# Spijkervet/Context-Aware-Sequential-Recommendation

Measured on AMD Instinct MI355X. Metric: user-sequences/sec (fwd+bwd), higher is better.
Workload: dtype f32 (bf16x3 split MFMA in attention); 1 GPU; ml-1m-shaped synthetic (6040 users, 3416 items), cast_1 maxlen=200 hidden_units=50 num_blocks=2 num_heads=1 dropout=0.20, batch 128/GPU (global 128), fwd+bwd+dense TF-Adam per step; parallelism=dp1, hip_graph=True, steps_per_graph_launch=4, attn_precision=bf16x3

## Files before the change

### context-aware-sequential-recommendation_amd/build.py

```python
import glob
import hashlib
import json
import os
import re
import subprocess
import sys
from concurrent.futures import ThreadPoolExecutor

PKG = os.path.dirname(os.path.abspath(__file__))
ROOT = os.path.dirname(PKG)
CSRC = os.path.join(PKG, "csrc")
LIB = os.path.join(PKG, "libcastrec.so")
LIB_TL = os.path.join(PKG, "libcastrec_tl.so")
SOURCES = ["cr_base.hip", "cr_embed.hip", "cr_layernorm.hip", "cr_eltwise.hip", "cr_gemm.hip",
           "cr_attn_fwd.hip", "cr_attn_bwd.hip", "cr_attn_bwd1.hip", "cr_attn_wide.hip", "cr_attn_bf.hip", "cr_gemm_bf.hip", "cr_block.hip", "cr_stack.hip", "cr_stack_bwd.hip", "cr_stack_bwd1.hip", "cr_wide.hip", "cr_head.hip", "cr_adam.hip", "cr_tgrad.hip", "cr_topk.hip", "cr_ce.hip", "cr_dist.hip", "cr_sampler.cpp", "cr_index.cpp"]
FLAGS = ["--offload-arch=gfx950", "-O3", "-fPIC", "-std=c++17", "-I", os.path.join(ROOT, "include"), "-I", CSRC,
         "-Wall", "-Wno-unused-function",
         "-fno-slp-vectorize"]


ISA_CHECKED = ["cr_stack.hip", "cr_stack_bwd.hip", "cr_stack_bwd1.hip", "cr_wide.hip", "cr_attn_bf.hip",
               "cr_block.hip", "cr_attn_fwd.hip", "cr_attn_bwd.hip", "cr_attn_bwd1.hip", "cr_gemm.hip", "cr_gemm_bf.hip",
               "cr_topk.hip", "cr_ce.hip"]
SLP_PROTECTED = ("cr_stack", "cr_wide")
_PK_F32 = ("v_pk_fma_f32", "v_pk_mul_f32", "v_pk_add_f32")
_LABEL = re.compile(r"^([A-Za-z_$][\w$.]*):")
_MODIFIER = re.compile(r"\s(op_sel|op_sel_hi|neg_lo|neg_hi|clamp|mul:|div:|quad_perm|row_|bank_mask|bound_ctrl|dst_sel|dst_unused|src\d_sel)")


def _operands(rest):
    m = _MODIFIER.search(" " + rest)
    if m:
        rest = (" " + rest)[:m.start()]
    return [o.strip().lstrip("-").strip("|") for o in rest.split(",") if o.strip()]


_VREG = re.compile(r"^v(?:\[(\d+):(\d+)\]|(\d+))$")
_WRITES_VGPR = ("v_", "ds_read", "global_load", "buffer_load", "flat_load", "scratch_load")


def _vregs(op):
    m = _VREG.match(op)
    if not m:
        return frozenset()
    if m.group(3) is not None:
        return frozenset([int(m.group(3))])
    return frozenset(range(int(m.group(1)), int(m.group(2)) + 1))


def scan_isa(text):
    out = dict(kernels=0, pk_fma=0, pk_add=0, pk_mul=0, in_place_any=0, mfma={}, mixed_mfma_chains=0, violations=[])
    func, last = "?", []
    mfma_dst = {}
    for no, line in enumerate(text.splitlines(), 1):
        if line and not line[0].isspace():
            m = _LABEL.match(line)
            if m and not line.startswith("."):
                func, last, mfma_dst = m.group(1), [], {}
                out["kernels"] += 1
            continue
        t = line.strip()
        if not t.startswith(_WRITES_VGPR):
            continue
        mn, _, rest = t.partition(" ")
        ops = _operands(rest.split(";")[0])
        dst = ops[0] if ops else ""
        dregs = _vregs(dst)
        if mn.startswith("v_mfma"):
            out["mfma"][mn] = out["mfma"].get(mn, 0) + 1
            srcc = _vregs(ops[3]) if len(ops) >= 4 else frozenset()
            prev = mfma_dst.get(srcc)
            if prev and prev[0] != mn:
                out["mixed_mfma_chains"] += 1
                out["violations"].append((func, no, [prev[1], t]))
            for k in [k for k in mfma_dst if k & dregs]:
                del mfma_dst[k]
            if dregs:
                mfma_dst[dregs] = (mn, t)
        elif dregs and mfma_dst:
            for k in [k for k in mfma_dst if k & dregs]:
                del mfma_dst[k]
        if not t.startswith("v_"):
            continue
        if mn in _PK_F32:
            out[mn[2:-4]] += 1
            if dst in ops[1:]:
                out["in_place_any"] += 1
            if mn == "v_pk_fma_f32" and len(ops) >= 4 and ops[3] == dst:
                for pm, pd, pl in last:
                    if pm in _PK_F32 and pd == dst:
                        out["violations"].append((func, no, [pl, t]))
                        break
        last = (last + [(mn, dst, t)])[-2:]
    return out


def _source_digest(src, headers, flags):
    h = hashlib.sha256()
    for f in [src] + headers:
        with open(f, "rb") as fh:
            h.update(fh.read())
    h.update(" ".join(flags).encode())
    return h.hexdigest()


def isa_summary_path(source_name, timeline=False):
    return os.path.join(CSRC, "build_tl" if timeline else "build", source_name + ".isa.json")


def check_isa_file(source_name, flags, headers, hipcc=None, listing=None):
    src = os.path.join(CSRC, source_name)
    if listing is None:
        listing = os.path.join(CSRC, "build", source_name + ".s")
        cmd = [hipcc or _hipcc()] + flags + ["-x", "hip", "-S", "--cuda-device-only", src, "-o", listing]
        r = subprocess.run(cmd, capture_output=True, text=True)
        if r.returncode != 0:
            raise RuntimeError("compile failed: %s\n%s" % (" ".join(cmd), r.stderr))
    with open(listing) as fh:
        res = scan_isa(fh.read())
    res["source"], res["digest"], res["flags"] = source_name, _source_digest(src, headers, flags), flags
    with open(isa_summary_path(source_name), "w") as fh:
        json.dump(res, fh, indent=1)
    if res["violations"]:
        f, no, chain = res["violations"][0]
        raise RuntimeError("%s: %d forbidden instruction chains in the device code (in-place packed fp32, or MFMAs of two shapes on one accumulator; first: %s, line %d: %s) -- see build.py ISA_CHECKED"
                           % (source_name, len(res["violations"]), f, no, " ; ".join(chain)))
    return res


def isa_is_current(source_name, flags, headers):
    try:
        with open(isa_summary_path(source_name)) as fh:
            d = json.load(fh)
    except (OSError, ValueError):
        return False
    return d.get("digest") == _source_digest(os.path.join(CSRC, source_name), headers, flags) and not d.get("violations")


def file_flags(source_name, timeline=False):
    extra = os.environ.get("CASTREC_EXTRA_FLAGS", "").split()
    slp_ok = os.environ.get("CASTREC_SLP_FILES", "cr_attn_bf.hip").split()
    bad = [f for f in slp_ok if f.startswith(SLP_PROTECTED)]
    if bad:
        raise RuntimeError("CASTREC_SLP_FILES names %s: these sources are never compiled with SLP vectorisation "
                           "(profiles/r04_flake/README.md)" % bad)
    if any(f in ("-fslp-vectorize", "-fvectorize-slp") or f.startswith("-fslp-vectorize") for f in extra):
        raise RuntimeError("CASTREC_EXTRA_FLAGS may not re-enable SLP vectorisation (profiles/r04_flake/README.md)")
    flags = FLAGS + (["-DCR_TIMELINE=1"] if timeline else []) + extra
    return [f for f in flags if not (f == "-fno-slp-vectorize" and source_name in slp_ok)]


HEADERS = [os.path.join(CSRC, h) for h in ("cr_common.hpp", "cr_attn_common.hpp", "cr_bf16.hpp", "cr_rlayout.hpp", "cr_rbwd.hpp")] \
    + [os.path.join(ROOT, "include", "castrec.h")]
EXTRA_DEPS = {"cr_adam.hip": ["cr_tgrad.hpp"], "cr_tgrad.hip": ["cr_tgrad.hpp"]}


def _hipcc():
    for c in (os.environ.get("HIPCC"), "/opt/rocm/bin/hipcc", "hipcc"):
        if c and (os.path.isabs(c) and os.path.exists(c) or not os.path.isabs(c)):
            return c
    raise RuntimeError("hipcc not found")


def _stale(obj, srcs):
    if not os.path.exists(obj):
        return True
    t = os.path.getmtime(obj)
    return any(os.path.getmtime(s) > t for s in srcs)


def build(force=False, verbose=False, timeline=False):
    hipcc = _hipcc()
    bdir = "build_tl" if timeline else "build"
    lib = LIB_TL if timeline else LIB
    os.makedirs(os.path.join(CSRC, bdir), exist_ok=True)
    headers = HEADERS
    objs, jobs = [], []
    for s in SOURCES:
        src = os.path.join(CSRC, s)
        obj = os.path.join(CSRC, bdir, s + ".o")
        objs.append(obj)
        fl = file_flags(s, timeline)
        checked = s in ISA_CHECKED and not timeline
        deps = [src] + headers + [os.path.join(CSRC, h) for h in EXTRA_DEPS.get(s, [])]
        if checked and not force and not _stale(obj, deps) and not isa_is_current(s, fl, headers):
            force_this = True
        else:
            force_this = False
        if force or force_this or _stale(obj, deps):
            cmd = [hipcc] + fl + (["-save-temps=obj"] if checked else []) + (["-x", "hip"] if s.endswith(".hip") else []) + ["-c", src, "-o", obj]
            jobs.append((cmd, s if checked else None, fl))

    def run(job):
        cmd, checked_src, fl = job if isinstance(job, tuple) else (job, None, None)
        r = subprocess.run(cmd, capture_output=True, text=True)
        if r.returncode != 0:
            raise RuntimeError("compile failed: %s\n%s\n%s" % (" ".join(cmd), r.stdout, r.stderr))
        if verbose and r.stderr.strip():
            print(r.stderr, file=sys.stderr)
        if checked_src:
            stem = checked_src[:-4]
            bd = os.path.join(CSRC, bdir)
            try:
                check_isa_file(checked_src, fl, headers, listing=os.path.join(bd, stem + "-hip-amdgcn-amd-amdhsa-gfx950.s"))
            finally:
                for f in glob.glob(os.path.join(bd, stem + "-hip-amdgcn-*")) + glob.glob(os.path.join(bd, stem + "-host-*")) \
                        + glob.glob(os.path.join(bd, stem + ".hip-hip-*")):
                    os.remove(f)

    with ThreadPoolExecutor(max_workers=4) as ex:
        list(ex.map(run, jobs))
    if force or jobs or _stale(lib, objs):
        run(([hipcc, "--offload-arch=gfx950", "-shared", "-fPIC", "-o", lib] + objs + ["-lpthread"], None, None))
    return lib


if __name__ == "__main__":
    print(build(force="--force" in sys.argv, verbose=True, timeline="--timeline" in sys.argv))
```

### context-aware-sequential-recommendation_amd/csrc/cr_adam.hip

```cpp
#include <math.h>
#include <stdlib.h>
#include <string.h>

#include "cr_common.hpp"
#include "cr_tgrad.hpp"

int tg_unit_grid(const cr_tgrad_desc* d);

#define ADAM_COLS 256
#define ADAM_WAVES 16
typedef float f4a __attribute__((ext_vector_type(4), aligned(4)));
__device__ __forceinline__ float slab_sum256(const float* slabs, int n_slabs, int n_dense, int j0, float (*part)[ADAM_COLS]) {
    const int lane = threadIdx.x & 63, w = threadIdx.x >> 6;
    const int j = j0 + 4 * lane;
    f4a acc = (f4a){0.f, 0.f, 0.f, 0.f};
    if (j + 3 < n_dense) {
        for (int s0 = w; s0 < n_slabs; s0 += 16 * ADAM_WAVES) {
            f4a v[16];
            int cnt = 0;
#pragma unroll
            for (int u = 0; u < 16; ++u)
                if (s0 + ADAM_WAVES * u < n_slabs) { v[u] = *reinterpret_cast<const f4a*>(slabs + (size_t)(s0 + ADAM_WAVES * u) * n_dense + j); cnt = u + 1; }
#pragma unroll
            for (int u = 0; u < 16; ++u)
                if (u < cnt) acc += v[u];
        }
    } else {
        for (int s = w; s < n_slabs; s += ADAM_WAVES)
            for (int u = 0; u < 4; ++u)
                if (j + u < n_dense) acc[u] += slabs[(size_t)s * n_dense + j + u];
    }
    part[w][4 * lane + 0] = acc.x; part[w][4 * lane + 1] = acc.y; part[w][4 * lane + 2] = acc.z; part[w][4 * lane + 3] = acc.w;
    __syncthreads();
    float g = 0.0f;
    if (threadIdx.x < ADAM_COLS) {
#pragma unroll
        for (int k = 0; k < ADAM_WAVES; ++k) g += part[k][threadIdx.x];
    }
    return g;
}

template <bool STREAM, int LPR, int VEC>
__global__ __launch_bounds__(64 * ADAM_WAVES) void k_adam(cr_adam_desc d, cr_tgrad_desc g, int nb_dense, int nb_lazy, int nb_units, int nb_ring) {
    __shared__ float part_s[ADAM_WAVES * ADAM_COLS + 4];
    float (*part)[ADAM_COLS] = reinterpret_cast<float (*)[ADAM_COLS]>(part_s);
    constexpr bool TG = LPR > 0;
    cr_kernarg_touch<sizeof(cr_adam_desc) + (TG ? sizeof(cr_tgrad_desc) : 0)>();
    const uint32_t t = d.step_snapshot ? *d.step_snapshot : *reinterpret_cast<const uint32_t*>(d.state + 4);
    const int bid = (int)blockIdx.x;
    if (bid >= (int)gridDim.x - nb_ring) {
        constexpr int NT = 64 * ADAM_WAVES;
        const long long n_copy = d.ids_copy_elems ? d.ids_copy_elems : d.ids_slot_elems;
        const int32_t* src1 = d.ids_ring + (long long)((t + 1u) % (uint32_t)d.ids_ring_slots) * d.ids_slot_elems;
        const long long first = (long long)(bid - ((int)gridDim.x - nb_ring)) * NT + threadIdx.x, stride = (long long)nb_ring * NT;
        if ((d.ids_slot_elems & 3) == 0 && (n_copy & 3) == 0 && (((uintptr_t)d.ids_ring | (uintptr_t)d.ids_dst) & 15) == 0) {
            const int4* src = reinterpret_cast<const int4*>(src1);
            int4* dst = reinterpret_cast<int4*>(d.ids_dst);
            for (long long i = first; i < (n_copy >> 2); i += stride) dst[i] = src[i];
        } else {
            for (long long i = first; i < n_copy; i += stride) d.ids_dst[i] = src1[i];
        }
        return;
    }
    const float* st = d.stats ? d.stats : d.state;
    const float n = st[2];
    float inv_n = 0.0f, lr_t = 0.0f;
    auto scalars = [&]() {
        inv_n = n > 0.0f ? 1.0f / n : 0.0f;
        const float b1t = powf(d.beta1, (float)t), b2t = powf(d.beta2, (float)t);
        lr_t = d.lr * sqrtf(1.0f - b2t) / (1.0f - b1t);
    };
    auto update = [&](long long i, float g) {
        g *= inv_n;
        if (i < d.n_l2) g = fmaf(d.l2, d.p[i], g);
        const float m = d.beta1 * d.m[i] + (1.0f - d.beta1) * g;
        const float v = d.beta2 * d.v[i] + (1.0f - d.beta2) * g * g;
        d.m[i] = m;
        d.v[i] = v;
        d.p[i] -= lr_t * m / (sqrtf(v) + d.eps);
    };
    if (bid < nb_dense) {
        const int j0 = bid * ADAM_COLS;
        const int ns = d.slab_counts ? min(d.slab_counts[bid], d.n_slabs) : d.n_slabs;
        const bool mine = threadIdx.x < ADAM_COLS && j0 + (int)threadIdx.x < d.n_dense;
        const long long i = d.n_table + j0 + (mine ? (int)threadIdx.x : 0);
        const float p0 = mine ? d.p[i] : 0.0f, m0 = mine ? d.m[i] : 0.0f, v0 = mine ? d.v[i] : 0.0f;
        float g = slab_sum256(d.dense_slabs, ns, d.n_dense, j0, part);
        scalars();
        if (mine) {
            g *= inv_n;
            if (i < d.n_l2) g = fmaf(d.l2, p0, g);
            const float m = d.beta1 * m0 + (1.0f - d.beta1) * g;
            const float v = d.beta2 * v0 + (1.0f - d.beta2) * g * g;
            d.m[i] = m;
            d.v[i] = v;
            d.p[i] = p0 - lr_t * m / (sqrtf(v) + d.eps);
        }
    } else if (bid < nb_dense + nb_lazy) {
        const int lane = threadIdx.x & 63;
        const int W = nb_lazy * ADAM_WAVES;
        scalars();
        for (int k = (bid - nb_dense) * ADAM_WAVES + (threadIdx.x >> 6); k < d.n_lazy_ids; k += W) {
            const int id = d.lazy_ids[k];
            if (id <= 0 || id >= d.lazy_rows) continue;
            int mine = 0;
            if (lane == 0) mine = atomicExch(&d.lazy_flags[id], t) != t;
            mine = __shfl(mine, 0, 64);
            if (!mine) continue;
            for (int c = lane; c < d.lazy_D; c += 64) {
                const long long i = (long long)id * d.lazy_D + c;
                const float g = d.table_grad[i];
                d.table_grad[i] = 0.0f;
                update(i, g);
            }
        }
    } else if (TG && bid < nb_dense + nb_lazy + nb_units) {
        const int32_t* ix = tg_index(g, t);
        constexpr int W = TG ? VEC : 1;
        scalars();
        tg_unit_blocks<TG ? LPR : 16, W, (TG && VEC == 4) ? 8 : 16>(g, ix, bid - nb_dense - nb_lazy, nb_units, part_s,
            reinterpret_cast<int*>(part_s + ADAM_WAVES * ADAM_COLS),
            [&](int row, int col0, const float (&acc)[W]) {
                const long long i = (long long)row * g.D + col0;
                float p0[W], m0[W], v0[W];
                tg_load<W>(p0, d.p + i); tg_load<W>(m0, d.m + i); tg_load<W>(v0, d.v + i);
#pragma unroll
                for (int u = 0; u < W; ++u) {
                    float gu = acc[u] * inv_n;
                    if (i + u < d.n_l2) gu = fmaf(d.l2, p0[u], gu);
                    m0[u] = d.beta1 * m0[u] + (1.0f - d.beta1) * gu;
                    v0[u] = d.beta2 * v0[u] + (1.0f - d.beta2) * gu * gu;
                    p0[u] -= lr_t * m0[u] / (sqrtf(v0[u]) + d.eps);
                }
                tg_store<W>(d.m + i, m0); tg_store<W>(d.v + i, v0); tg_store<W>(d.p + i, p0);
            });
    } else if (TG) {
        const int32_t* ix = tg_index(g, t);
        const uint32_t* bits = reinterpret_cast<const uint32_t*>(ix + ix[6]);
        const int nb_table = gridDim.x - nb_dense - nb_lazy - nb_units - nb_ring;
        const int tb = bid - nb_dense - nb_lazy - nb_units;
        constexpr int NT = 64 * ADAM_WAVES;
        const long long stride = (long long)nb_table * NT;
        auto touched = [&](uint32_t row) { return ((bits[row >> 5] >> (row & 31)) & 1u) != 0u; };
        scalars();
        if ((g.D & 3) == 0) {
            const float b1 = d.beta1, b2 = d.beta2, c1 = 1.0f - d.beta1, c2 = 1.0f - d.beta2;
            auto ld4 = [](const float* q) { return STREAM ? __builtin_nontemporal_load(reinterpret_cast<const f4a*>(q)) : *reinterpret_cast<const f4a*>(q); };
            auto st4 = [](float* q, const f4a x) {
                if (STREAM) __builtin_nontemporal_store(x, reinterpret_cast<f4a*>(q));
                else *reinterpret_cast<f4a*>(q) = x;
            };
            const long long n4 = d.n_table >> 2;
            const unsigned D4 = (unsigned)g.D >> 2;
            const int sh = (D4 & (D4 - 1u)) == 0u ? __builtin_ctz(D4) : -1;
            constexpr int U = 4;
            for (long long q = (long long)tb * NT + threadIdx.x; q < n4; q += U * stride) {
                bool in[U];
                uint32_t bw[U];
                uint32_t row[U];
                f4a p[U], m[U], v[U];
#pragma unroll
                for (int u = 0; u < U; ++u) {
                    const long long qq = q + u * stride;
                    in[u] = qq < n4;
                    const long long qc = in[u] ? qq : q;
                    row[u] = sh >= 0 ? (uint32_t)(qc >> sh) : (uint32_t)((unsigned long long)qc / D4);
                    bw[u] = bits[row[u] >> 5];
                    p[u] = ld4(d.p + 4 * qc); m[u] = ld4(d.m + 4 * qc); v[u] = ld4(d.v + 4 * qc);
                }
#pragma unroll
                for (int u = 0; u < U; ++u) {
                    if (!in[u] || ((bw[u] >> (row[u] & 31)) & 1u)) continue;
                    const long long i = 4 * (q + u * stride);
                    f4a po;
#pragma unroll
                    for (int e = 0; e < 4; ++e) {
                        float gu = 0.0f;
                        if (i + e < d.n_l2) gu = fmaf(d.l2, p[u][e], gu);
                        m[u][e] = b1 * m[u][e] + c1 * gu;
                        v[u][e] = b2 * v[u][e] + c2 * gu * gu;
                        po[e] = p[u][e] - lr_t * m[u][e] / (sqrtf(v[u][e]) + d.eps);
                    }
                    st4(d.m + i, m[u]); st4(d.v + i, v[u]); st4(d.p + i, po);
                }
            }
        } else {
            for (long long i = (long long)tb * NT + threadIdx.x; i < d.n_table; i += stride)
                if (!touched((uint32_t)((unsigned long long)i / (unsigned)g.D))) update(i, 0.0f);
        }
    } else {
        const int nb_table = gridDim.x - nb_dense - nb_lazy - nb_ring;
        const int tb = bid - nb_dense - nb_lazy;
        const long long first = nb_lazy > 0 ? (long long)d.lazy_rows * d.lazy_D : 0;
// ... 189 lines not shown
```

### context-aware-sequential-recommendation_amd/csrc/cr_stack_bwd1.hip

```cpp
#include <math.h>
#include <stdlib.h>
#include <string.h>
#include <type_traits>
#include <mutex>

#include "cr_rbwd.hpp"

#define B1_DRAIN() asm volatile("s_waitcnt vmcnt(0)" ::: "memory")
#define B1_NT_WS true
#define B1_ROWS 224
#define B1_FSTR (B1_ROWS * 64)

#define DS_EXACT(DS) ((DS) > 0 ? ((DS) & 255) : (DS))
#define DS_D(DS, run) ((DS) > 0 ? ((DS) & 255) : (run))
#define B1_NKT(DS, a) ((DS) > 255 ? (((DS) >> 8) & 255) : (a).nkt)
#define B1_T(DS, a) ((DS) > 65535 ? ((DS) >> 16) : (a).T)
#undef D_NF
#define D_NF(DS) ((DS) > 0 ? ((DS) & 255) / 16 : ((DS) < 0 ? -(DS) - 1 : -1))

struct B1Args {
    cr_block_bwd_desc bd;
    cr_attn_desc ad;
    cr_embed_bwd_desc sc;
    cr_ln_bwd_desc ln;
    const float* dy2;
    float* dx2;
    const float* ln_dy2;
    float* d_addend2;
    float* sbuf; float* sbuf2;
    int B, T, nkt, scatter, has_ln;
    int small;
    int n0, add;
    float isd, isd_log2e, invT;
    unsigned qpk[8], kpk[8];
    unsigned long long* ts;
};

__device__ __forceinline__ const B1Args& b1_args_again() {
    auto p = __builtin_amdgcn_kernarg_segment_ptr();
    asm volatile("" : "+s"(p));
    return *reinterpret_cast<const B1Args*>((const void*)p);
}

#ifdef CR_TIMELINE
#define B1_TS(slot)                                                                                          \
    do {                                                                                                     \
        if (a.ts && (threadIdx.x & 63) == 0) {                                                               \
            unsigned long long* ts_ = a.ts + (((size_t)blockIdx.y * gridDim.x + blockIdx.x) * SB_WAVES + (threadIdx.x >> 6)) * 32; \
            ts_[(slot)] = ((slot) == 0 || (slot) == 31) ? wall_clock64() : clock64();                        \
            if ((slot) == 0) ts_[30] = clock64();          \
            if ((slot) == 31) ts_[29] = clock64();                                                           \
        }                                                                                                    \
    } while (0)
#else
#define B1_TS(slot) do { } while (0)
#endif

template <bool SPLIT>
struct B1Lds {
    static constexpr int NIMG = SPLIT ? 4 : 2;
    static constexpr int WST = SPLIT ? 2 * ST_WIMG : ST_WIMG;
    static constexpr int IST = SPLIT ? 2 * SB_IMG : SB_IMG;
    static constexpr int MATB = (SPLIT ? 2 : 1) * B1_FSTR * 2;
    static constexpr int LOB = B1_FSTR * 2;
    static constexpr int W_OFF = NIMG * B1_FSTR;
    static constexpr int F_OFF_BYTES = (W_OFF + 2 * WST) * 2;
    static constexpr int GAM = 0, GAMF = 64, PART = 128, PARTF = PART + 2 * SB_WAVES * 64, SDEL = PARTF + 2 * SB_WAVES * 64,
                         KB = SDEL + 2 * B1_ROWS, SMX = KB, SUNI = SMX + 2 * B1_ROWS, SQV = SUNI + B1_ROWS,
                         TFLAG = SQV + B1_ROWS, NFLOAT = TFLAG + 16;
    static_assert(SUNI >= KB + B1_ROWS + 16, "the key bias (one extra tile) inside the shared floats");
    static constexpr int BYTES = F_OFF_BYTES + NFLOAT * 4;
};

template <bool BIAS = false>
__device__ __forceinline__ void b1_wstore(float* dst, int ldw, float* bias_dst, const f32x4 (&acc)[2], const f32x4 (&accb)[2], int D, int it, int jt0, bool add) {
    const int lane = threadIdx.x & 63, li = lane & 15, lg = lane >> 4;
#pragma unroll
    for (int j = 0; j < 2; ++j) {
        const int col = 16 * (jt0 + j) + li;
#pragma unroll
        for (int r = 0; r < 4; ++r) {
            const int k = 16 * it + 4 * lg + r;
            if (col < D && (BIAS ? k < D : k <= D)) {
                float* p = (k < D) ? dst + (size_t)k * ldw + col : bias_dst + col;
                __builtin_nontemporal_store(add ? *p + acc[j][r] : acc[j][r], p);
            }
        }
        if (BIAS && it == 0 && lg == 0 && col < D) bias_dst[col] = add ? bias_dst[col] + accb[j][0] : accb[j][0];
    }
}
__device__ __forceinline__ void b1_ln_fold(float* part, const f32x4 (&ag)[4], const f32x4 (&ab)[4]) {
    const int lane = lane_now(), wave = __builtin_amdgcn_readfirstlane(threadIdx.x >> 6), lg = lane >> 4;
    float u[16];
#pragma unroll
    for (int ct = 0; ct < 4; ++ct)
#pragma unroll
        for (int r = 0; r < 4; ++r) {
            float x = ag[ct][r];
            asm volatile("s_nop 1\n\t"
                         "v_add_f32_dpp %0, %0, %0 row_mirror row_mask:0xf bank_mask:0x3\n\t"
                         "v_add_f32_dpp %0, %1, %1 row_mirror row_mask:0xf bank_mask:0xc"
                         : "+v"(x) : "v"(ab[ct][r]));
            u[4 * ct + r] = x;
        }
#pragma unroll
    for (int j = 0; j < 8; ++j)
        asm volatile("s_nop 1\n\t"
                     "v_add_f32_dpp %0, %0, %0 row_half_mirror row_mask:0xf bank_mask:0x5\n\t"
                     "v_add_f32_dpp %0, %1, %1 row_half_mirror row_mask:0xf bank_mask:0xa"
                     : "+v"(u[j]) : "v"(u[8 + j]));
    const bool b1 = (lane & 2) != 0, b0 = (lane & 1) != 0;
    float w[4], z[2];
#pragma unroll
    for (int j = 0; j < 4; ++j) {
        const float keep = b1 ? u[4 + j] : u[j], send = b1 ? u[j] : u[4 + j];
        w[j] = keep + __int_as_float(__builtin_amdgcn_update_dpp(0, __float_as_int(send), 0x1B, 0xF, 0xF, false));
    }
#pragma unroll
    for (int j = 0; j < 2; ++j) {
        const float keep = b0 ? w[2 + j] : w[j], send = b0 ? w[j] : w[2 + j];
        z[j] = keep + __int_as_float(__builtin_amdgcn_update_dpp(0, __float_as_int(send), 0xB1, 0xF, 0xF, false));
    }
    const int col = 16 * (((lane >> 2) & 1) * 2 + ((lane >> 1) & 1)) + 4 * lg + 2 * (lane & 1);
    float* dst = part + ((lane & 8) ? SB_WAVES * 64 : 0) + wave * 64 + col;
    *reinterpret_cast<float2*>(dst) = make_float2(z[0], z[1]);
}
template <int NSET = 1>
__device__ __forceinline__ void b1_ln_flush(const float* part, float* dg, float* db, int D, bool add) {
    for (int c = threadIdx.x; c < D; c += SB_NT) {
        float g = 0.0f, b = 0.0f;
#pragma unroll
        for (int s = 0; s < NSET; ++s)
#pragma unroll
            for (int w = 0; w < SB_WAVES; ++w) { g += part[(2 * s * SB_WAVES + w) * 64 + c]; b += part[((2 * s + 1) * SB_WAVES + w) * 64 + c]; }
        dg[c] = add ? dg[c] + g : g;
        db[c] = add ? db[c] + b : b;
    }
}

struct B1Steps { uint32_t ffn2, attn, emb; };
struct B1Acc { f32x4 aw1[2], aw2[2], aw1b[2], aw2b[2], ag[4], ab[4], agF[4], abF[4]; };

template <bool SPLIT, int DS, bool QSIDE, int HD, class F>
__device__ __forceinline__ void b1_phase1(const B1Args& a, unsigned char* smem, int n, B1Acc& A, B1Steps& steps, F&& before_last_products) {
    constexpr bool BIAS = DS_EXACT(DS) == 64;
    constexpr bool LATE_Q = !QSIDE && (HD == 2 || DS_EXACT(DS) > 50 || DS <= 0);
    typedef B1Lds<SPLIT> L;
    const cr_block_bwd_desc& bd = a.bd;
    const cr_block_desc& d = bd.f;
    __bf16* Im = reinterpret_cast<__bf16*>(smem);
    __bf16* Wi = Im + L::W_OFF;
    float* fl = reinterpret_cast<float*>(smem + L::F_OFF_BYTES);
    float* gam = fl + L::GAM; float* gamF = fl + L::GAMF; float* part = fl + L::PART; float* partF = fl + L::PARTF; float* sdel = fl + L::SDEL;
    constexpr int WST = L::WST, IST = L::IST;
    const int D = DS_D(DS, d.D), T = B1_T(DS, a);
    const DCtx dcx = d_ctx<D_NF(DS)>(D);
    const int wave = __builtin_amdgcn_readfirstlane(threadIdx.x >> 6);
    uint32_t sv_ffn2 = cr_step_request(d.drop_ffn2), sv_attn = cr_step_request(a.ad.drop), sv_emb = a.scatter ? cr_step_request(a.sc.f.drop) : 0u;
    const float scale1 = (d.drop_ffn1.rate > 0.0f) ? 1.0f / (1.0f - d.drop_ffn1.rate) : 1.0f;
    B1_TS(13);
    f32x4 (&aw1)[2] = A.aw1; f32x4 (&aw2)[2] = A.aw2; f32x4 (&ag)[4] = A.ag; f32x4 (&ab)[4] = A.ab; f32x4 (&agF)[4] = A.agF; f32x4 (&abF)[4] = A.abF;
    f32x4 (&aw1b)[2] = A.aw1b; f32x4 (&aw2b)[2] = A.aw2b;
#pragma unroll
    for (int j = 0; j < 2; ++j) { aw1[j] = (f32x4){0.f, 0.f, 0.f, 0.f}; aw2[j] = aw1[j]; aw1b[j] = aw1[j]; aw2b[j] = aw1[j]; }
#pragma unroll
    for (int ct = 0; ct < 4; ++ct) { ag[ct] = (f32x4){0.f, 0.f, 0.f, 0.f}; ab[ct] = ag[ct]; agF[ct] = ag[ct]; abF[ct] = ag[ct]; }
    const int it = wave >> 1, jt0 = 2 * (wave & 1);
    RRaw rdy, rdy2, rhid, rfin, ro, rq, ry;
    const size_t MD = (size_t)d.M * D;
    auto tile_rows = [&](int rd, int& m, bool& rok) {
        const int q = 16 * (rd * SB_TPR + wave) + (lane_now() & 15);
        rok = q < T;
        m = n * T + min(q, T - 1);
    };
    auto issue_a = [&](int rd) {
        if (rd * SB_TPR < B1_NKT(DS, a) && wave < min(SB_TPR, B1_NKT(DS, a) - rd * SB_TPR)) {
            int m; bool rok;
            tile_rows(rd, m, rok);
            const u32 mo = (u32)m * (u32)(4 * D);
            if (a.has_ln) {
                r_issue(rdy, a.ln.dy, (u32)m * (u32)(4 * a.ln.lddy), dcx, rok);
                if (a.ln_dy2) r_issue(rdy2, a.ln_dy2, (u32)m * (u32)(4 * a.ln.lddy), dcx, rok);
                r_issue(ry, d.y, mo, dcx);
            } else {
                r_issue(rdy, bd.dy, mo, dcx);
                if (a.dy2) r_issue(rdy2, a.dy2, mo, dcx);
            }
            r_issue(rhid, d.hid, mo, dcx);
// ... 849 lines not shown
                    d4[t2] = *reinterpret_cast<const float4*>(vq + 64 * t2 + 4 * B1_ROWS * h);
                    w4[t2] = *reinterpret_cast<const float4*>(vq + 64 * t2 + 4 * (L::SQV - L::SDEL));
                }
                constexpr int JB = (SPLIT || HD == 2) ? 2 : 4;
                const int jbase = HD == 2 ? 2 * h : 0;
                bf8 oth[JB], otl[JB];
#pragma unroll
                for (int jt = 0; jt < JB; ++jt) {
                    oth[jt] = trF(L::MATB, jbase + jt, 0);
                    otl[jt] = SPLIT ? trF(L::MATB, jbase + jt, 1) : oth[jt];
                }
                float xa[8], xd[8];
                const uint32_t xb_h = xbase + (uint32_t)h * xhead;
                auto finish = [&](auto diag_c, int t2, int xo, const f32x4& s, const f32x4& p) {
                    constexpr bool DIAG = decltype(diag_c)::value;
                    const int lt = 2 * qp + t2;
                    const float mm[4] = {m4[t2].x, m4[t2].y, m4[t2].z, m4[t2].w}, dd[4] = {d4[t2].x, d4[t2].y, d4[t2].z, d4[t2].w}, ww[4] = {w4[t2].x, w4[t2].y, w4[t2].z, w4[t2].w};
                    const uint32_t x0 = xb_h + (uint32_t)lt * (16u * xT);
                    const float bias = (lt < kt) ? -INFINITY : kbias;
                    float pn[4], w[4];
#pragma unroll
                    for (int r = 0; r < 4; ++r) {
                        pn[r] = __builtin_amdgcn_exp2f(fmaf(s[r], a.isd_log2e, -mm[r]) + bias);
                        if (DIAG) pn[r] = (lt != kt || key <= 16 * lt + 4 * lg + r) ? pn[r] : 0.0f;
                        w[r] = (cr_mix(x0 + (uint32_t)r * xT) >= dc.thresh) ? ww[r] : 0.0f;
                        xd[xo + r] = pn[r] * (p[r] * w[r] - dd[r]);
                    }
                    if ((uni_m >> lt) & 1u) {
                        const float4 u4 = *reinterpret_cast<const float4*>(vq + 64 * t2 + 4 * (L::SUNI - L::SDEL));
                        const float uu[4] = {u4.x, u4.y, u4.z, u4.w};
#pragma unroll
                        for (int r = 0; r < 4; ++r) xa[xo + r] = (pn[r] + key_in_T * uu[r]) * w[r];
                    } else {
#pragma unroll
                        for (int r = 0; r < 4; ++r) xa[xo + r] = pn[r] * w[r];
                    }
                };
                if (qp == (kt >> 1)) {
                    finish(std::true_type{}, 0, 0, s0, p0);
                    finish(std::true_type{}, 1, 4, s1, p1);
                } else {
                    finish(std::false_type{}, 0, 0, s0, p0);
                    finish(std::false_type{}, 1, 4, s1, p1);
                }
                bf8 ah, al, dh, dl;
                split8<SPLIT>(xa, ah, al);
                split8<SPLIT>(xd, dh, dl);
#pragma unroll
                for (int jt = 0; jt < JB; ++jt) dv[jbase + jt] = mma<SPLIT>(oth[jt], otl[jt], ah, al, dv[jbase + jt]);
                if (HD == 1) {
#pragma unroll
                    for (int j0 = JB; j0 < 4; j0 += JB) {
#pragma unroll
                        for (int jt = 0; jt < JB; ++jt) {
                            oth[jt] = trF(L::MATB, j0 + jt, 0);
                            otl[jt] = SPLIT ? trF(L::MATB, j0 + jt, 1) : oth[jt];
                        }
#pragma unroll
                        for (int jt = 0; jt < JB; ++jt) dv[j0 + jt] = mma<SPLIT>(oth[jt], otl[jt], ah, al, dv[j0 + jt]);
                        BF_SGB(0x100, (SPLIT ? 4 : 2) * JB, 0);
                        BF_SGB(0x008, (SPLIT ? 3 : 1) * JB, 0);
                    }
                }
#pragma unroll
                for (int j0 = jbase; j0 < (HD == 2 ? jbase + 2 : 4); j0 += JB) {
#pragma unroll
                    for (int jt = 0; jt < JB; ++jt) {
                        oth[jt] = trF(0, j0 + jt, 0);
                        otl[jt] = SPLIT ? trF(0, j0 + jt, 1) : oth[jt];
                    }
#pragma unroll
                    for (int jt = 0; jt < JB; ++jt) dk[j0 + jt] = mma<SPLIT>(oth[jt], otl[jt], dh, dl, dk[j0 + jt]);
                    BF_SGB(0x100, (SPLIT ? 4 : 2) * JB, 0);
                    BF_SGB(0x008, (SPLIT ? 3 : 1) * JB, 0);
                }
            }
        }
#pragma unroll
        for (int jt = 0; jt < 4; ++jt) dk[jt] *= a.isd;
        if (ti == 0) B1_TS(6);
        if (ti == 0 && (int)((tpk >> 5) & 31u) < B1_NKT(DS, a)) issue_tile((int)((tpk >> 5) & 31u));
        const B1Args& ar = b1_args_again();
        r_store<B1_NT_WS>(const_cast<float*>(ar.bd.dqkv) + MD, mo, dk, rok, dcx);
        r_store<B1_NT_WS>(const_cast<float*>(ar.bd.dqkv) + 2 * MD, mo, dv, rok, dcx);
        f32x4 dxp[4];
        {
            bf8 gh[2], gl[2];
            r_split<SPLIT>(dk, gh, gl);
            r_gemm_t<SPLIT, false>(dxp, Wi, Wi + ST_WIMG, gh, gl);
            r_split<SPLIT>(dv, gh, gl);
            r_gemm_t<SPLIT, true>(dxp, Wi + WST, Wi + WST + ST_WIMG, gh, gl);
        }
        if (ar.scatter) {
            b1_scatter_prep(ar, dxp, m, rok, D, steps.emb);
            r_store(ar.sbuf2, mo, dxp, rok, dcx);
        } else {
            r_store(ar.dx2, mo, dxp, rok, dcx);
        }
    }
    B1_TS(4);
    __builtin_amdgcn_s_setprio(0);
    B1_DRAIN();
    __syncthreads();
    B1_TS(7);
    f32x4 awk[2], awv[2], awkb[2], awvb[2];
#pragma unroll
    for (int j = 0; j < 2; ++j) { awk[j] = (f32x4){0.f, 0.f, 0.f, 0.f}; awv[j] = awk[j]; awkb[j] = awk[j]; awvb[j] = awk[j]; }
    const int it = wave >> 1, jt0 = 2 * (wave & 1);
    const int R = B1_NKT(DS, a) > SB_TPR ? 2 : 1;
    RRaw r1, r2, r3;
    auto issue3 = [&](int rd) {
        if (rd < R && wave < min(SB_TPR, B1_NKT(DS, a) - rd * SB_TPR)) {
            const int qq = 16 * (rd * SB_TPR + wave) + (lane_now() & 15);
            const u32 mo = (u32)(base_row + min(qq, T - 1)) * (u32)(4 * D);
            r_issue(r1, bk.x, mo, dcx);
            r_issue(r2, dKg, mo, dcx, qq < T);
            r_issue(r3, dVg, mo, dcx, qq < T);
        }
    };
    issue3(0);
    B1Small small;
#pragma unroll 1
    for (int rd = 0; rd < R; ++rd) {
        const int ntr = min(SB_TPR, B1_NKT(DS, a) - rd * SB_TPR);
        if (wave < ntr) {
            f32x4 x[4], g[4];
            r_finish(x, r1, dcx);
            plant_one(x, D);
            img_put<SPLIT>(Im, Im + SB_IMG, 16 * wave, x);
            r_finish(g, r2, dcx);
            img_put<SPLIT>(Im + IST, Im + IST + SB_IMG, 16 * wave, g);
            r_finish(g, r3, dcx);
            img_put<SPLIT>(Im + 2 * IST, Im + 2 * IST + SB_IMG, 16 * wave, g);
        }
        issue3(rd + 1);
        if (rd == R - 1 && a.scatter && a.small) b1_small_issue<D_NF(DS)>(small, a, a.sbuf2, n, D);
        __syncthreads();
        if (rd == 0) B1_TS(16);
        wgrad_accum<SPLIT, BIAS>(awk, awkb, Im, Im + SB_IMG, Im + IST, Im + IST + SB_IMG, ntr, it, jt0);
        wgrad_accum<SPLIT, BIAS>(awv, awvb, Im, Im + SB_IMG, Im + 2 * IST, Im + 2 * IST + SB_IMG, ntr, it, jt0);
        __syncthreads();
        if (rd == 0) B1_TS(19);
    }
    B1_TS(17);
    const size_t so = (size_t)blockIdx.x * bd.slab_stride;
    b1_wstore<BIAS>(bd.g_wqkv + so + D, 3 * D, bd.g_bqkv + so + D, awk, awkb, D, it, jt0, add);
    b1_wstore<BIAS>(bd.g_wqkv + so + 2 * D, 3 * D, bd.g_bqkv + so + 2 * D, awv, awvb, D, it, jt0, add);
    B1_TS(18);
    if (a.scatter && a.small) b1_small_table<SPLIT, D_NF(DS)>(a, smem, reinterpret_cast<int*>(fl + L::PART), small, n, D, add);
    else if (a.scatter) b1_scatter_rows(a, a.sbuf2, n, D);
    B1_TS(5);
}

template <bool SPLIT, int DS, int HD>
__global__ __launch_bounds__(SB_NT) void k_stack_block_bwd(B1Args a) {
    extern __shared__ __attribute__((aligned(16))) unsigned char smem_raw[];
    B1_TS(0);
    cr_kernarg_touch<sizeof(B1Args)>();
    B1_TS(15);
    const int n = a.n0 + (int)blockIdx.x;
    if (blockIdx.y == 0) {
        B1Acc acc;
        B1Steps steps;
        b1_phase1<SPLIT, DS, false, HD>(a, smem_raw, n, acc, steps, [] {});
        b1_k_side<SPLIT, DS, HD>(a, smem_raw, n, a.add != 0, acc, steps);
    } else {
        B1Acc acc;
        B1Stage st;
        WRegs<1, SB_NT> w;
        B1Steps steps;
        b1_phase1<SPLIT, DS, true, HD>(a, smem_raw, n, acc, steps, [&] { b1_q_stage_issue<DS>(a, n, st, w); });
        b1_q_side<SPLIT, DS, HD>(a, smem_raw, n, a.add != 0, acc, steps, st, w);
    }
    B1_TS(31);
}

struct B1Deal { unsigned pk[8]; bool done; };
static void b1_deal_search(int nkt, bool query_pass, unsigned (&pk)[8]) {
    int wave_of[16], order[16];
    cr_deal_search(nkt, query_pass, wave_of, order);
    for (int w = 0; w < 8; ++w) pk[w] = 0x3FFu;
    int wc[8] = {0, 0, 0, 0, 0, 0, 0, 0};
    for (int k = 0; k < nkt; ++k) {
        const int t = order[k], w = wave_of[t];
        pk[w] = (pk[w] & ~(31u << (5 * wc[w]))) | ((unsigned)t << (5 * wc[w]));
        ++wc[w];
    }
}
static void b1_deal_tiles(int nkt, bool query_pass, unsigned (&pk)[8]) {
    static B1Deal cache[2][16];
    static std::mutex mu;
    {
        std::lock_guard<std::mutex> lock(mu);
        B1Deal& c = cache[query_pass ? 1 : 0][nkt & 15];
        if (!c.done) { b1_deal_search(nkt, query_pass, c.pk); c.done = true; }
        for (int w = 0; w < 8; ++w) pk[w] = c.pk[w];
    }
    if (const char* ov = getenv(query_pass ? "CASTREC_B1_QPK" : "CASTREC_B1_KPK")) {
        unsigned t[8];
        int w = 0;
        const char* c = ov;
        while (w < 8 && *c) {
            unsigned a0 = 31, a1 = 31;
            if (*c != '-') { a0 = (unsigned)strtol(c, const_cast<char**>(&c), 10); if (*c == ':') { ++c; a1 = (unsigned)strtol(c, const_cast<char**>(&c), 10); } }
            else ++c;
            t[w++] = (a0 & 31u) | ((a1 & 31u) << 5);
            if (*c == ',') ++c;
        }
        if (w == 8) for (int i = 0; i < 8; ++i) pk[i] = t[i];
    }
}

extern "C" int cr_stack_block_bwd_deal(int nkt, int query_pass, uint32_t* pk) {
    CR_REQUIRE(pk && nkt >= 1 && nkt <= 2 * SB_TPR, "cr_stack_block_bwd_deal: 1 <= tiles <= 14");
    unsigned t[8];
    b1_deal_tiles(nkt, query_pass != 0, t);
    for (int w = 0; w < 8; ++w) pk[w] = t[w];
    return CR_OK;
}

static const char* b1_unsupported(const cr_block_bwd_desc* bd, const cr_attn_desc* ad, int B, int T, int precision) {
    if (!bd || !ad) return "NULL description";
    const cr_block_desc& d = bd->f;
    const bool two_heads = d.D == 64 && ad->H == 2 && ad->d == 32;
    if (!two_heads && (d.D < 8 || d.D >= 64)) return "hidden size 8..63 (one head), or 64 with two heads of 32";
    if (precision != CR_PREC_BF16X3 && precision != CR_PREC_BF16) return "bf16 arithmetic (precision) only";
    if (B < 1 || T < 1 || d.M != B * T) return "M = B T";
    if ((T + 15) / 16 > 2 * SB_TPR) return "T <= 224 (two rounds of 7 row tiles)";
    if ((size_t)d.M * d.D * 4 >= ((size_t)1 << 32)) return "activations of 4 GiB or more (32-bit row offsets)";
    if (bd->n_slabs < 1) return "n_slabs";
    if (!two_heads && (ad->H != 1 || ad->d != d.D)) return "one head of d = D (or two heads of 32 at D = 64)";
    if (ad->B != B || ad->T != T) return "the block's B and T";
    if (ad->ld != d.D || ad->Q != d.qkv || ad->K != d.qkv + (size_t)d.M * d.D || ad->V != d.qkv + 2 * (size_t)d.M * d.D) return "Q / K / V = the parts of the block's qkv";
    if (ad->residual != d.q_in || ad->out != d.o || ad->k_valid != d.k_valid || ad->q_valid != d.q_valid) return "the attention call of this block (residual = q_in, out = o, masks)";
    if (!ad->row_stats) return "row_stats (saved by the forward)";
    if (ad->attn_weights) return "attention weights are not taken";
    return nullptr;
}
extern "C" int cr_stack_block_bwd_supported(const cr_block_bwd_desc* bd, const cr_attn_desc* ad, int B, int T, int precision) {
    return b1_unsupported(bd, ad, B, T, precision) == nullptr;
}

template <bool SPLIT, int DS, int HD = 1>
static int launch_b1(B1Args& a, int nwg, hipStream_t s) {
    static cr_devmask attr = 0;
    int rc = cr_raise_lds_limit(reinterpret_cast<const void*>(&k_stack_block_bwd<SPLIT, DS, HD>), &attr);
    if (rc) return rc;
    for (int n0 = 0; n0 < a.B; n0 += nwg) {
        a.n0 = n0;
        a.add = n0 > 0;
        hipLaunchKernelGGL((k_stack_block_bwd<SPLIT, DS, HD>), dim3(a.B - n0 < nwg ? a.B - n0 : nwg, 2), dim3(SB_NT), B1Lds<SPLIT>::BYTES, s, a);
    }
    return cr_check_launch("cr_stack_block_bwd");
}

extern "C" int cr_stack_block_bwd(const cr_block_bwd_desc* bd, const cr_attn_desc* ad, const cr_block_bwd1_ext* x, const cr_ln_bwd_desc* lnf,
                                  const cr_embed_bwd_desc* sc, int B, int T, int precision, void* stream) {
    const char* why = b1_unsupported(bd, ad, B, T, precision);
    CR_REQUIRE(why == nullptr, "cr_stack_block_bwd: unsupported (%s)", why ? why : "");
    CR_REQUIRE(x != nullptr, "cr_stack_block_bwd: NULL extension");
    B1Args a;
    memset(static_cast<void*>(&a), 0, sizeof(a));
    a.bd = *bd; a.ad = *ad;
    a.B = B; a.T = T; a.nkt = (T + 15) / 16;
    const cr_block_desc* d = &bd->f;
    CR_REQUIRE(bd->d_o && bd->dqkv && d->hid && d->f_in && d->o && d->q_in && d->x && d->mask_ids && d->w1 && d->w2 && d->wqkv && d->ln1_g && d->ln2_g,
               "cr_stack_block_bwd: NULL pointer");
    CR_REQUIRE(bd->g_w1 && bd->g_b1 && bd->g_w2 && bd->g_b2 && bd->g_ln2_g && bd->g_ln2_b && bd->g_wqkv && bd->g_bqkv && bd->g_ln1_g && bd->g_ln1_b,
               "cr_stack_block_bwd: NULL gradient pointer");
    CR_REQUIRE(bd->dq_part == nullptr, "cr_stack_block_bwd: dq_part is not taken");
    a.dy2 = x->dy2; a.dx2 = x->dx2; a.ln_dy2 = x->lnf_dy2; a.d_addend2 = x->d_addend2;
    if (lnf) {
        CR_REQUIRE(lnf->x == d->y && lnf->ldx == d->D && lnf->M == d->M && lnf->D == d->D, "cr_stack_block_bwd: the LayerNorm's input must be this block's y");
        CR_REQUIRE(lnf->gamma && lnf->dy && lnf->dgamma && lnf->dbeta && lnf->accumulate == 0, "cr_stack_block_bwd: LayerNorm backward arguments");
        CR_REQUIRE(lnf->slab_stride == bd->slab_stride && lnf->n_slabs == bd->n_slabs, "cr_stack_block_bwd: the LayerNorm's slabs must be the block's");
        CR_REQUIRE((size_t)lnf->M * lnf->lddy * 4 < ((size_t)1 << 32), "cr_stack_block_bwd: dy of 4 GiB or more");
        a.ln = *lnf;
        a.has_ln = 1;
    } else {
        CR_REQUIRE(bd->dy, "cr_stack_block_bwd: dy is NULL");
        CR_REQUIRE(x->lnf_dy2 == nullptr, "cr_stack_block_bwd: lnf_dy2 without a LayerNorm");
    }
    if (sc) {
        const cr_embed_desc* e = &sc->f;
        CR_REQUIRE(e->ids && e->M == d->M && e->D == d->D && e->ld_out == d->D && e->col_off == 0 && e->T > 0 && e->V > 0,
                   "cr_stack_block_bwd: the embedding recipe must describe the block's dense input x");
        CR_REQUIRE(!bd->dx_accumulate, "cr_stack_block_bwd: dx_accumulate with a scatter (this kernel must be the only producer of dx)");
        if (sc->n_slabs > 0) {
            const int nw = B < bd->n_slabs ? B : bd->n_slabs;
            CR_REQUIRE(sc->table_grad && !sc->pos_grad && e->V <= 256 && sc->n_slabs >= 2 * nw,
                       "cr_stack_block_bwd: small-table scatter needs table_grad, no pos_grad, V <= 256 and n_slabs >= 2 * min(B, n_slabs of the block)");
            a.small = 1;
        }
        CR_REQUIRE(sc->d_addend == nullptr || (e->ld_add == d->D && x->d_addend2 != nullptr), "cr_stack_block_bwd: d_addend must be dense [M, D] and come with d_addend2");
        a.sc = *sc;
        a.scatter = 1;
        a.sbuf = sc->d_addend ? sc->d_addend : bd->dx;
        a.sbuf2 = sc->d_addend ? x->d_addend2 : x->dx2;
        CR_REQUIRE(a.sbuf && a.sbuf2 && a.sbuf != a.sbuf2, "cr_stack_block_bwd: the scatter needs two [M, D] row buffers (d_addend + d_addend2, or dx + dx2)");
    } else {
        CR_REQUIRE(bd->dx && x->dx2 && bd->dx != x->dx2, "cr_stack_block_bwd: dx / dx2");
    }
    a.isd = 1.0f / sqrtf((float)ad->d);
    a.isd_log2e = a.isd * 1.4426950408889634f;
    a.invT = 1.0f / (float)T;
    b1_deal_tiles(a.nkt, true, a.qpk);
    b1_deal_tiles(a.nkt, false, a.kpk);
    a.ts = g_attn_ts_which == 9 ? g_attn_ts : nullptr;
    if (a.ts) {
        static const char* only = getenv("CASTREC_TS_LAUNCH");
        static unsigned long long* seen_for = nullptr;
        static int count = 0;
        if (seen_for != a.ts) { seen_for = a.ts; count = 0; }
        if (only && atoi(only) != count) a.ts = nullptr;
        ++count;
    }
    const int nwg = B < bd->n_slabs ? B : bd->n_slabs;
    const bool split = precision == CR_PREC_BF16X3;
    hipStream_t s = cr_stream(stream);
    switch (d->D) {
    case 64: return split ? launch_b1<true, 64, 2>(a, nwg, s) : launch_b1<false, 64, 2>(a, nwg, s);
    case 50:
        static const bool no_nk = getenv("CASTREC_B1_NO_NKT") != nullptr;
        if (a.T == 200 && !no_nk) return split ? launch_b1<true, 50 | (13 << 8) | (200 << 16)>(a, nwg, s) : launch_b1<false, 50 | (13 << 8) | (200 << 16)>(a, nwg, s);
        return split ? launch_b1<true, 50>(a, nwg, s) : launch_b1<false, 50>(a, nwg, s);
    case 32: return split ? launch_b1<true, 32>(a, nwg, s) : launch_b1<false, 32>(a, nwg, s);
    case 40: return split ? launch_b1<true, 40>(a, nwg, s) : launch_b1<false, 40>(a, nwg, s);
    case 48: return split ? launch_b1<true, 48>(a, nwg, s) : launch_b1<false, 48>(a, nwg, s);
    case 56: return split ? launch_b1<true, 56>(a, nwg, s) : launch_b1<false, 56>(a, nwg, s);
    default: break;
    }
    switch (d->D / 16) {
    case 0: return split ? launch_b1<true, -1>(a, nwg, s) : launch_b1<false, -1>(a, nwg, s);
    case 1: return split ? launch_b1<true, -2>(a, nwg, s) : launch_b1<false, -2>(a, nwg, s);
    case 2: return split ? launch_b1<true, -3>(a, nwg, s) : launch_b1<false, -3>(a, nwg, s);
    default: return split ? launch_b1<true, -4>(a, nwg, s) : launch_b1<false, -4>(a, nwg, s);
    }
}
```

### context-aware-sequential-recommendation_amd/engine.py

```python
import ctypes as C
import math
import os
import zlib

import numpy as np
import torch

from . import lib as L
from . import ops as O

ATTN_PRECISIONS = {"f32": L.PREC_F32, "bf16x3": L.PREC_BF16X3, "bf16": L.PREC_BF16}
DEFAULT_ATTN_PRECISION = "bf16x3"
LOSSES = ("bce", "ce")
ALL_LOSSES = LOSSES + ("sampled_ce", "gbce")
SOFTMAX_LOSSES = ("ce", "sampled_ce", "gbce")
SAMPLED_LOSSES = ("sampled_ce", "gbce")
CE_PROPOSALS = ("uniform", "popularity")

MODELS = ["cast_1", "cast_2", "cast_3", "cast_4", "cast_5", "cast_6", "cast_7", "cast_8", "cast_9",
          "sasrec", "sasrec_static"]


def site_id(name):
    return zlib.crc32(name.encode()) & 0xFFFFFF


def positional_encoding(dim, length):
    v = np.array([pos / np.power(10000, 2 * i / dim) for pos in range(length) for i in range(dim)])
    v[::2] = np.sin(v[::2])
    v[1::2] = np.cos(v[1::2])
    return v.reshape(length, dim).astype(np.float32)


class Hyper:

    def __init__(self, args=None, **kw):
        d = dict(maxlen=50, hidden_units=50, num_blocks=2, num_heads=1, dropout_rate=0.5, l2_emb=0.0, lr=1e-3,
                 max_bins=200, num_context_blocks=2, seed=42, loss="bce", ce_negatives=256, gbce_t=0.75, ce_proposal="uniform",
                 ce_pop_power=1.0)
        for k in d:
            if args is not None and hasattr(args, k):
                d[k] = getattr(args, k)
        d.update(kw)
        self.__dict__.update(d)
        if self.hidden_units % self.num_heads != 0:
            raise ValueError("hidden_units must be divisible by num_heads (tf.split, modules.py:208)")


def auto_slabs(M):
    n = -(-M // 128)
    if n < 128:
        n = -(-M // 64)
    return max(1, min(256, n))


def _stack_entries(prefix, L_, D):
    out = []
    for i in range(L_):
        p = "%s.%d." % (prefix, i)
        out += [(p + "ln1.gamma", (D,), "ones"), (p + "ln1.beta", (D,), "zeros"),
                (p + "wqkv", (D, 3 * D), "glorot3"), (p + "bqkv", (3 * D,), "zeros"),
                (p + "ln2.gamma", (D,), "ones"), (p + "ln2.beta", (D,), "zeros"),
                (p + "w1", (D, D), "glorot"), (p + "b1", (D,), "zeros"),
                (p + "w2", (D, D), "glorot"), (p + "b2", (D,), "zeros")]
    out += [(prefix + ".lnf.gamma", (D,), "ones"), (prefix + ".lnf.beta", (D,), "zeros")]
    return out


def model_structure(model, hp):
    L_, Lc = hp.num_blocks, hp.num_context_blocks
    s = dict(ctx={}, small=[], mlp=0, learned_pos=model in ("sasrec", "cast_9"))
    if model in ("cast_1", "cast_2", "cast_3", "cast_4", "cast_5", "cast_6"):
        s["ctx"]["ctx_time"] = L_
    if model == "cast_8":
        s["ctx"].update(ctx_hours=L_, ctx_days=L_)
    if model == "cast_9":
        s["ctx"].update(ctx_hours=Lc, ctx_days=Lc, ctx_time=Lc)
    if "ctx_time" in s["ctx"]:
        s["small"].append(("time_emb", hp.max_bins + 1))
    if model in ("cast_3", "cast_4", "cast_5", "cast_6", "cast_7", "cast_8", "cast_9"):
        s["small"] += [("hours_emb", 25), ("days_emb", 8)]
    s["mlp"] = {"cast_2": 2, "cast_3": 3, "cast_4": 4, "cast_5": 3, "cast_6": 4, "cast_7": 3, "cast_8": 3, "cast_9": 4}.get(model, 0)
    return s


class ParamLayout:
    def __init__(self, model, usernum, itemnum, hp):
        D, T = hp.hidden_units, hp.maxlen
        st = model_structure(model, hp)
        table = [("item_emb", (itemnum + 1, D), "glorot")]
        if st["learned_pos"]:
            table.append(("pos_emb", (T, D), "glorot"))
        dense = [(n, (v, D), "glorot") for n, v in st["small"]]
        for pfx, Lc in st["ctx"].items():
            dense += _stack_entries(pfx, Lc, D)
        if st["mlp"]:
            k = st["mlp"]
            dense += [("mlp.w1", (k * D, k * D), "glorot"), ("mlp.b1", (k * D,), "zeros"),
                      ("mlp.w2", (k * D, D), "glorot"), ("mlp.b2", (D,), "zeros")]
        dense += _stack_entries("trunk", hp.num_blocks, D)
        self.entries, off = {}, 0
        for (n, shape, init) in table:
            self.entries[n] = (off, shape, init, "table"); off += int(np.prod(shape))
        self.n_table = off
        for (n, shape, init) in dense:
            self.entries[n] = (off, shape, init, "dense"); off += int(np.prod(shape))
        self.n_total, self.n_dense, self.D = off, off - self.n_table, D
        self.n_l2 = self.n_table + sum(int(np.prod(self.entries[n][1])) for n, _ in st["small"])

    def logical_names(self):
        out = []
        for n in self.entries:
            if n.endswith("wqkv"):
                out += [n[:-4] + x for x in ("wq", "wk", "wv")]
            elif n.endswith("bqkv"):
                out += [n[:-4] + x for x in ("bq", "bk", "bv")]
            else:
                out.append(n)
        return out

    def view(self, flat, name):
        D = self.D
        for j, x in enumerate(("q", "k", "v")):
            if name.endswith(".w" + x):
                off, shape, _, _ = self.entries[name[:-2] + "wqkv"]
                return flat[off:off + D * 3 * D].view(D, 3 * D)[:, j * D:(j + 1) * D]
            if name.endswith(".b" + x):
                off, shape, _, _ = self.entries[name[:-2] + "bqkv"]
                return flat[off + j * D:off + (j + 1) * D]
        off, shape, _, _ = self.entries[name]
        return flat[off:off + int(np.prod(shape))].view(*shape)

    def init_host(self, seed):
        rs = np.random.RandomState(seed)
        flat = np.zeros(self.n_total, np.float32)
        for n, (off, shape, init, _) in self.entries.items():
            size = int(np.prod(shape))
            if init == "glorot":
                lim = math.sqrt(6.0 / (shape[0] + shape[1]))
                flat[off:off + size] = rs.uniform(-lim, lim, size)
            elif init == "glorot3":
                D = shape[0]
                lim = math.sqrt(6.0 / (D + D))
                flat[off:off + size] = rs.uniform(-lim, lim, size)
            elif init == "ones":
                flat[off:off + size] = 1.0
        return flat


class Engine:
    def __init__(self, model, usernum, itemnum, hp, batch_size, training=True, seed=None, n_slabs=None,
                 share=None, batch_global=None, row_offset=0, want_attn=False, device="cuda", fused=None,
                 attn_precision=None, lazy_adam=None, loss=None, ce_negatives=None, gbce_t=None, ce_proposal=None):
        if model not in MODELS:
            raise ValueError("model must be one of %s" % MODELS)
        if not torch.cuda.is_available():
            raise RuntimeError("castrec_amd needs a ROCm GPU (gfx950); there is no CPU fallback")
        self.model, self.hp, self.B, self.T, self.D = model, hp, batch_size, hp.maxlen, hp.hidden_units
        self.H = hp.num_heads
        if attn_precision is None:
            attn_precision = os.environ.get("CASTREC_ATTN_PRECISION") or getattr(hp, "attn_precision", None) or DEFAULT_ATTN_PRECISION
        if attn_precision not in ATTN_PRECISIONS:
            raise ValueError("attn_precision must be one of %s" % sorted(ATTN_PRECISIONS))
        self.attn_precision = attn_precision
        if attn_precision == "f32" and hp.hidden_units > 64:
            import warnings
            warnings.warn("attn_precision='f32' at hidden_units %d leaves the tuned path: the exact-fp32 row phases above 64 columns are "
                          "the unfused kernels (2.6x slower at the C4 shape, 11x at C5; profiles/r02d_other_shapes.log); the "
                          "fp32-grade default is 'bf16x3'" % hp.hidden_units, RuntimeWarning, stacklevel=2)
        self.lazy_adam = bool(int(os.environ.get("CASTREC_LAZY_ADAM", "0"))) if lazy_adam is None else bool(lazy_adam)
        if loss is None:
            loss = getattr(hp, "loss", None) or "bce"
        if loss not in ALL_LOSSES:
            raise ValueError("loss must be one of %s, got %r" % (ALL_LOSSES, loss))
        self.loss = loss if training else "bce"
        if ce_negatives is None:
            ce_negatives = getattr(hp, "ce_negatives", None) or 256
        self.ce_negatives = int(ce_negatives)
        if gbce_t is None:
            gbce_t = getattr(hp, "gbce_t", None)
            gbce_t = 0.75 if gbce_t is None else gbce_t
        self.gbce_t = float(gbce_t)
        if ce_proposal is None:
            ce_proposal = getattr(hp, "ce_proposal", None) or "uniform"
        if ce_proposal not in CE_PROPOSALS:
            raise ValueError("ce_proposal must be one of %s, got %r" % (CE_PROPOSALS, ce_proposal))
        self.ce_proposal = ce_proposal if training else "uniform"
        if self.ce_proposal == "popularity" and self.loss != "sampled_ce":
            raise ValueError("ce_proposal='popularity' needs loss='sampled_ce', got loss=%r (gbce's beta is derived for uniform "
                             "sampling; bce and ce draw no shared negatives)" % self.loss)
        if self.loss in SOFTMAX_LOSSES:
            op = {"ce": "cr_softmax_ce", "sampled_ce": "cr_sampled_ce", "gbce": "cr_gbce"}[self.loss]
            if self.lazy_adam:
                raise ValueError("loss='%s' does not take row-sparse Adam (lazy_adam): every item row has a gradient" % self.loss)
            if (batch_global is not None and batch_global != batch_size) or row_offset:
                raise ValueError("loss='%s' does not take data parallelism (the item table's gradient is not in the exchanged bucket)"
                                 % self.loss)
            if not 8 <= hp.hidden_units <= 256:
                raise ValueError("loss='%s' needs 8 <= hidden_units <= 256 (%s), got %d" % (self.loss, op, hp.hidden_units))
        if self.loss in SAMPLED_LOSSES and not 1 <= self.ce_negatives <= L.CR_SCE_MAX_SAMPLES:
            raise ValueError("loss='%s' needs 1 <= ce_negatives <= %d (%s), got %d"
                             % (self.loss, L.CR_SCE_MAX_SAMPLES, op, self.ce_negatives))
        if self.loss == "gbce":
            if not 0.0 <= self.gbce_t <= 1.0:
                raise ValueError("loss='gbce' needs 0 <= gbce_t <= 1, got %r" % (gbce_t,))
            alpha = min(1.0, self.ce_negatives / max(1, itemnum - 1))
            self.gbce_beta = 1.0 - self.gbce_t * (1.0 - alpha)
        self.M = self.B * self.T
        self.usernum, self.itemnum = usernum, itemnum
        self.training = training
        self.single_pass_bwd = os.environ.get("CASTREC_TWO_PASS_ATTN_BWD") != "1"
        self.fuse_tails = os.environ.get("CASTREC_NO_TAILS") != "1"
        self.fuse_embed = os.environ.get("CASTREC_NO_EMBED_FUSION") != "1"
        self.fuse_stack = os.environ.get("CASTREC_NO_STACK_KERNEL") != "1"
        self.fuse_stack_bwd = os.environ.get("CASTREC_NO_STACK_BWD") != "1"
        self.fuse_wide = os.environ.get("CASTREC_NO_WIDE") != "1"
        self._pending_embed = {}
        self._scatter_recipe, self._scatter_claimed = {}, set()
        self._ln_recipe, self._ln_claimed = {}, set()
        self._lnf_intent = {}
        self.fuse_block_bwd = os.environ.get("CASTREC_NO_BLOCK_BWD") != "1"
        self._grad2 = {}
        self._grad2_bufs = {}
        self._block_bwd_ranges = []
        self.fuse_head_ln = os.environ.get("CASTREC_NO_HEAD_LN") != "1" and self.loss == "bce"
        self._check_ids = os.environ.get("CASTREC_NO_ID_CHECK") != "1"
        self.fused = (4 <= hp.hidden_units <= 64) if fused is None else bool(fused)
        if self.fused and not 4 <= hp.hidden_units <= 64:
            raise ValueError("fused block kernels need 4 <= hidden_units <= 64")
        self.dev = torch.device(device)
        self.seed = hp.seed if seed is None else seed
        self.layout = share.layout if share is not None else ParamLayout(model, usernum, itemnum, hp)
        lay = self.layout
        if not n_slabs:
            n_slabs = auto_slabs(batch_size * hp.maxlen)
            if (self.fused and self.attn_precision != "f32" and 8 <= self.D <= 64 and self.T <= 224
                    and os.environ.get("CASTREC_NO_STACK_BWD") != "1"):
                items = batch_size * (2 if self.T > 112 else 1)
                if n_slabs < items <= 512:
                    n_slabs = items
                if (training and self.T > 16 and batch_size <= 160 and n_slabs < 2 * batch_size <= 512
                        and os.environ.get("CASTREC_NO_HEAD_FUSION") != "1"):
                    n_slabs = 2 * batch_size
        self.n_slabs = n_slabs
        self.n_wslabs = n_slabs if (self.fused or self.D <= 128) else min(n_slabs, int(os.environ.get("CASTREC_WSLABS", "32")))
        self._wgrad_ranges = []
        self.slab_counts = None
        f32 = dict(dtype=torch.float32, device=self.dev)
        if share is not None:
            self.P = share.P
        else:
            self.P = torch.from_numpy(lay.init_host(self.seed)).to(self.dev)
        self.state = torch.zeros(L.CR_STATE_FLOATS, **f32)
        self.state[4:5].view(torch.int32)[0] = 1
        if training:
            self.Mom = torch.zeros(lay.n_total, **f32)
            self.Vel = torch.zeros(lay.n_total, **f32)
            self.Gflat = torch.zeros(lay.n_total + 4, **f32)
            self.Gt = self.Gflat[:lay.n_table]
            self.Gs = torch.zeros(n_slabs, max(lay.n_dense, 1), **f32)
            if self.loss in SOFTMAX_LOSSES:
                nb = (O.softmax_ce_workspace_bytes(self.M, itemnum + 1, self.D) if self.loss == "ce"
                      else O.sampled_ce_workspace_bytes(self.M, self.ce_negatives, self.D) if self.loss == "sampled_ce"
                      else O.gbce_workspace_bytes(self.M, self.ce_negatives, self.D))
                self._ce_ws = torch.empty(nb, dtype=torch.uint8, device=self.dev)
            if self.loss in SAMPLED_LOSSES:
                self.samples = torch.zeros(self.ce_negatives, dtype=torch.int32, device=self.dev)
            if self.ce_proposal == "popularity":
                self.item_cdf = torch.zeros(itemnum + 1, dtype=torch.int32, device=self.dev)
                self.item_logq = torch.zeros(itemnum + 1, **f32)
                self._have_item_weights = False
        self.drop = O.Drop(hp.dropout_rate if training else 0.0, self.seed, self.state, row_offset)
        self.batch_global = self.B if batch_global is None else batch_global
        self.want_attn = want_attn
        self.attn_weights = None
        self._bufs, self._keep = {}, []
        self.fwd, self.bwd = [], []
        self._bwd_factories = []
        self._grad_written = set()
        i32 = dict(dtype=torch.int32, device=self.dev)
        self.ID_KEYS = ("seq", "pos", "neg", "time", "hours", "days")
        ng, ent = C.c_int(0), C.c_int(0)
        self.use_index = bool(training and not self.lazy_adam and self.loss == "bce" and os.environ.get("CASTREC_NO_INDEX") != "1"
                              and L.lib.cr_tgrad_geometry(self.D, C.byref(ng), C.byref(ent)))
        self.ids_words = 6 * self.M
        self.index_off = (self.ids_words + 3) // 4 * 4
        self.index_lay, self._ixb = None, None
        if self.use_index:
            self.index_lay = L.IndexLayout()
            t_pos = self.T if "pos_emb" in self.layout.entries else 0
            L.check(L.lib.cr_batch_index_layout(self.M, itemnum + 1, t_pos, ng.value, ent.value, C.byref(self.index_lay)), "cr_batch_index_layout")
            self._ixb = L.lib.cr_index_builder_create(self.M, itemnum + 1, t_pos, ng.value, ent.value)
            if not self._ixb:
                raise MemoryError("cr_index_builder_create(%d, %d, %d)" % (self.M, itemnum + 1, t_pos))
            self._tg_part = torch.zeros(self.index_lay.cap_blocks, (self.D + 3) // 4 * 4, dtype=torch.float32, device=self.dev)
            self._tg_tickets = torch.zeros(self.index_lay.cap_blocks, dtype=torch.int32, device=self.dev)
        self.slot_words = self.index_off + (int(self.index_lay.total_words) if self.use_index else 0) if self.use_index else self.ids_words
        self.batch_buf = torch.zeros(self.slot_words, **i32)
        self.ids_all = self.batch_buf[:self.ids_words].view(6, self.M)
        self.ids = {k: self.ids_all[i] for i, k in enumerate(self.ID_KEYS)}
        self._host_slot = np.zeros(self.slot_words, np.int32)
        self._tg_rows = None
        self.bitwise_reproducible = self.use_index
        self.static_pe = torch.from_numpy(positional_encoding(self.D, self.T)).to(self.dev)
        self._build()
        self._finalize()
        self.graph = None
        self._id_ring, self._ring_next = None, None

    def buf(self, name, cols, rows=None):
        if name not in self._bufs:
            self._bufs[name] = torch.zeros(self.M if rows is None else rows, cols, dtype=torch.float32, device=self.dev)
        return self._bufs[name]

    def vec(self, name, n=None):
        if name not in self._bufs:
            self._bufs[name] = torch.zeros(self.M if n is None else n, dtype=torch.float32, device=self.dev)
        return self._bufs[name]

    def p(self, name):
        return self.layout.view(self.P, name)

    def _pptr(self, name):
        off = self.layout.entries[name][0]
        return self.P.data_ptr() + 4 * off

    def _gptr(self, name):
        off, _, _, kind = self.layout.entries[name]
        if kind == "table":
            return self.Gt.data_ptr() + 4 * off
        return self.Gs.data_ptr() + 4 * (off - self.layout.n_table)

    def _acc(self, key):
        first = key not in self._grad_written
        self._grad_written.add(key)
        return 0 if first else 1

    def _call(self, lst, name, *args):
        if name in ("cr_gemm_rows", "cr_gemm_wgrad"):
            for i in range(args[1]):
                args[0][i].precision = ATTN_PRECISIONS[self.attn_precision]
        if name == "cr_gemm_wgrad":
            args = args[:3] + (self.n_wslabs,)
            base = self.Gs.data_ptr()
            for i in range(args[1]):
                w = args[0][i]
                o = (w.dW - base) // 4
                self._wgrad_ranges += [(o + k * w.ldw, o + k * w.ldw + w.N) for k in range(w.K)]
                if w.db:
                    self._wgrad_ranges.append(((w.db - base) // 4, (w.db - base) // 4 + w.N))
        fn = getattr(L.lib, name)
        self._keep.append(args)
        lst.append((name, fn, args))

    def rng(self, site_name, enabled=True):
        return self.drop.rng(site_id(site_name), enabled and self.training)

    def op_embed(self, ids_key, table, out, ld_out, col_off, scale, pos=None, addend=None, drop_site=None,
                 mask=False, small=False, into_stack=False):
        V, D = self.layout.entries[table][1]
        pos_ptr = None
        if pos == "static":
            pos_ptr = self.static_pe.data_ptr()
        elif pos == "learned":
            pos_ptr = self._pptr("pos_emb")
        add_buf = addend[0] if addend else None
        d = L.EmbedDesc(self.ids[ids_key].data_ptr(), self._pptr(table), self.M, self.T, D, V, 1, float(scale), pos_ptr,
                        add_buf.data_ptr() if addend else None, add_buf.shape[1] if addend else 0,
                        self.rng(drop_site) if drop_site else O.NO_DROP,
                        self.ids["seq"].data_ptr() if mask else None, out.data_ptr(), ld_out, col_off)
        if into_stack and self.fused and self.fuse_embed and ld_out == D and col_off == 0:
            self._pending_embed[out.data_ptr()] = d
        else:
            self._call(self.fwd, "cr_embed_fwd", C.byref(d))
        if not self.training:
            return

# ... 209 lines not shown
                G = self._gptr
                bbd = L.BlockBwdDesc(L.BlockDesc.from_buffer_copy(wbd), dy.data_ptr(), do.data_ptr(), dqkv.data_ptr(), dx.data_ptr(),
                                     self._acc(id(dx)), G(pfx + "ln1.gamma"), G(pfx + "ln1.beta"), G(pfx + "wqkv"), G(pfx + "bqkv"),
                                     G(pfx + "ln2.gamma"), G(pfx + "ln2.beta"), G(pfx + "w1"), G(pfx + "b1"), G(pfx + "w2"), G(pfx + "b2"),
                                     S, self.n_slabs)
                own_w = D == 128 and os.environ.get("CASTREC_WIDE_NO_WGRAD") != "1"
                if not own_w:
                    bbd.g_w1 = bbd.g_b1 = bbd.g_w2 = bbd.g_b2 = bbd.g_wqkv = bbd.g_bqkv = None
                dh = D // H
                fuse_attn = (T <= 256 and 8 <= dh <= 64 and dh % 16 == 0 and os.environ.get("CASTREC_WIDE_NO_DELTA") != "1"
                             and os.environ.get("CASTREC_BF_TWO_KERNELS") is None)
                if fuse_attn:
                    delta = self.vec("attn_delta_heads", H * M)
                    bbd.attn_delta = delta.data_ptr()
                self._call(lst, "cr_wide_ln_ffn_bwd", C.byref(bbd), g2.data_ptr(), g1.data_ptr(), H if fuse_attn else 0, prec)
                if not own_w:
                    w = (L.WgradDesc * 2)(L.WgradDesc(hid.data_ptr(), D, g2.data_ptr(), D, G(pfx + "w2"), D, G(pfx + "b2"), M, D, D),
                                          L.WgradDesc(f_in.data_ptr(), D, g1.data_ptr(), D, G(pfx + "w1"), D, G(pfx + "b1"), M, D, D))
                    self._call(lst, "cr_gemm_wgrad", w, 2, S, self.n_slabs)
                dq, dk, dv = dqkv.data_ptr(), dqkv.data_ptr() + MD4, dqkv.data_ptr() + 2 * MD4
                abd = L.AttnBwdDesc(L.AttnDesc.from_buffer_copy(ad), do.data_ptr(), D, dq, dk, dv, D, stats.data_ptr())
                if fuse_attn:
                    abd.delta = delta.data_ptr()
                self._call(lst, "cr_attn_bwd", C.byref(abd))
                if not own_w:
                    gw, gb = G(pfx + "wqkv"), G(pfx + "bqkv")
                    w2 = (L.WgradDesc * 3)(L.WgradDesc(q_in.data_ptr(), D, dq, D, gw, 3 * D, gb, M, D, D),
                                           L.WgradDesc(x.data_ptr(), D, dk, D, gw + 4 * D, 3 * D, gb + 4 * D, M, D, D),
                                           L.WgradDesc(x.data_ptr(), D, dv, D, gw + 8 * D, 3 * D, gb + 8 * D, M, D, D))
                    self._call(lst, "cr_gemm_wgrad", w2, 3, S, self.n_slabs)
                self._call(lst, "cr_wide_ln_qkv_bwd", C.byref(bbd), prec)
                return lst
            e = L.EltDesc(L.ELT_GRADPREP, dy.data_ptr(), D, None, 0, g2.data_ptr(), D, M, D, self.rng(pfx[:-1] + ".ffn2"), ids.data_ptr(), 0)
            self._call(lst, "cr_eltwise", C.byref(e))
            b = O.gemm_desc(g2, D, None, D, g1, D, M, D, D, trans_b=True)
            b.B = self._pptr(pfx + "w2")
            self._call(lst, "cr_gemm_rows", (L.GemmDesc * 1)(b), 1)
            e1 = L.EltDesc(L.ELT_GRADPREP, g1.data_ptr(), D, hid.data_ptr(), D, g1.data_ptr(), D, M, D, self.rng(pfx[:-1] + ".ffn1"), None, 0)
            self._call(lst, "cr_eltwise", C.byref(e1))
            w = (L.WgradDesc * 2)(L.WgradDesc(hid.data_ptr(), D, g2.data_ptr(), D, self._gptr(pfx + "w2"), D, self._gptr(pfx + "b2"), M, D, D),
                                  L.WgradDesc(f_in.data_ptr(), D, g1.data_ptr(), D, self._gptr(pfx + "w1"), D, self._gptr(pfx + "b1"), M, D, D))
            self._call(lst, "cr_gemm_wgrad", w, 2, S, self.n_slabs)
            b1 = O.gemm_desc(g1, D, None, D, df, D, M, D, D, trans_b=True, residual=dy, ldr=D, mask_ids=ids)
            b1.B = self._pptr(pfx + "w1")
            self._call(lst, "cr_gemm_rows", (L.GemmDesc * 1)(b1), 1)
            l2 = L.LnBwdDesc(o.data_ptr(), D, self._pptr(pfx + "ln2.gamma"), df.data_ptr(), D, do.data_ptr(), D, 0,
                             self._gptr(pfx + "ln2.gamma"), self._gptr(pfx + "ln2.beta"), S, self.n_slabs, M, D, 1e-8)
            self._call(lst, "cr_layernorm_bwd", C.byref(l2))
            dq, dk, dv = dqkv.data_ptr(), dqkv.data_ptr() + MD4, dqkv.data_ptr() + 2 * MD4
            abd = L.AttnBwdDesc(L.AttnDesc.from_buffer_copy(ad), do.data_ptr(), D, dq, dk, dv, D, stats.data_ptr())
            self._call(lst, "cr_attn_bwd", C.byref(abd))
            gw = self._gptr(pfx + "wqkv"); gb = self._gptr(pfx + "bqkv")
            w2 = (L.WgradDesc * 3)(L.WgradDesc(q_in.data_ptr(), D, dq, D, gw, 3 * D, gb, M, D, D),
                                   L.WgradDesc(x.data_ptr(), D, dk, D, gw + 4 * D, 3 * D, gb + 4 * D, M, D, D),
                                   L.WgradDesc(x.data_ptr(), D, dv, D, gw + 8 * D, 3 * D, gb + 8 * D, M, D, D))
            self._call(lst, "cr_gemm_wgrad", w2, 3, S, self.n_slabs)
            bq = O.gemm_desc(None, D, None, 3 * D, dq_in, D, M, D, D, trans_b=True, residual=do, ldr=D)
            bq.A, bq.B = dq, wqkv
            bk = O.gemm_desc(None, D, None, 3 * D, dx, D, M, D, D, trans_b=True, accumulate=bool(self._acc(id(dx))))
            bk.A, bk.B = dk, wqkv + 4 * D
            self._call(lst, "cr_gemm_rows", (L.GemmDesc * 2)(bq, bk), 2)
            bv = O.gemm_desc(None, D, None, 3 * D, dx, D, M, D, D, trans_b=True, accumulate=True)
            bv.A, bv.B = dv, wqkv + 8 * D
            self._call(lst, "cr_gemm_rows", (L.GemmDesc * 1)(bv), 1)
            l1 = L.LnBwdDesc(x.data_ptr(), D, self._pptr(pfx + "ln1.gamma"), dq_in.data_ptr(), D, dx.data_ptr(), D, 1,
                             self._gptr(pfx + "ln1.gamma"), self._gptr(pfx + "ln1.beta"), S, self.n_slabs, M, D, 1e-8)
            self._call(lst, "cr_layernorm_bwd", C.byref(l1))
            return lst
        self._bwd_factories.append(factory)

    def _block_desc(self, x, y, pfx):
        M, D = self.M, self.D
        q_in, o, f_in, hid = (self.buf(pfx + n, D) for n in ("q_in", "o", "f_in", "hid"))
        qkv = self.buf(pfx + "qkv", D, rows=3 * M)
        kvalid, qvalid = self.vec(pfx + "kvalid"), self.vec(pfx + "qvalid")
        P = self._pptr
        return L.BlockDesc(M, D, P(pfx + "ln1.gamma"), P(pfx + "ln1.beta"), P(pfx + "wqkv"), P(pfx + "bqkv"),
                           P(pfx + "ln2.gamma"), P(pfx + "ln2.beta"), P(pfx + "w1"), P(pfx + "b1"), P(pfx + "w2"), P(pfx + "b2"),
                           x.data_ptr(), q_in.data_ptr(), qkv.data_ptr(), kvalid.data_ptr(), qvalid.data_ptr(), o.data_ptr(),
                           f_in.data_ptr(), hid.data_ptr(), y.data_ptr(), self.ids["seq"].data_ptr(),
                           self.rng(pfx[:-1] + ".ffn1"), self.rng(pfx[:-1] + ".ffn2"))

    def _op_block_fused(self, x, y, pfx, attn_out, q_in, o, f_in, hid, qkv, kvalid, qvalid, skip_qkv=False, tail=None,
                        collect=None):
        M, D, H, B, T = self.M, self.D, self.H, self.B, self.T
        ids = self.ids["seq"]
        bd = self._block_desc(x, y, pfx)
        if not skip_qkv and collect is None:
            e = self._pending_embed.pop(x.data_ptr(), None)
            if e is not None:
                self._keep.append(e)
                self._call(self.fwd, "cr_block_ln_qkv_fwd_gather", C.byref(bd), C.byref(e))
            else:
                self._call(self.fwd, "cr_block_ln_qkv_fwd", C.byref(bd))
        MD4 = 4 * M * D
        ad = O.attn_desc(qkv, None, None, D, kvalid, qvalid, q_in, D, o, D, B, T, H, D // H,
                         rng=self.rng(pfx + "attn"), batch_global=self.batch_global,
                         dead_ids=None if attn_out is not None else ids, attn_weights=attn_out)
        ad.K, ad.V = qkv.data_ptr() + MD4, qkv.data_ptr() + 2 * MD4
        ad.precision = ATTN_PRECISIONS[self.attn_precision]
        bf = ad.precision != L.PREC_F32 and 8 <= D // H <= 64 and T <= 1024
        one_pass = self.training and H == 1 and self.single_pass_bwd and not bf
        if one_pass or (self.training and bf):
            row_stats = self.vec(pfx + "row_stats", H * B * T * 4)
            ad.row_stats = row_stats.data_ptr()
        if collect is not None:
            collect.append((bd, ad))
        else:
            self._call(self.fwd, "cr_attn_fwd", C.byref(ad))
        if collect is not None:
            pass
        elif tail is None:
            self._call(self.fwd, "cr_block_ln_ffn_fwd", C.byref(bd))
        elif tail[0] == "next":
            nbd = self._block_desc(y, tail[2], tail[1])
            td = L.BlockTailDesc(1, C.pointer(nbd), None, None, None, 0, 0)
            self._keep.append(nbd)
            self._call(self.fwd, "cr_block_ln_ffn_fwd_tail", C.byref(bd), C.byref(td))
        else:
            _, pname, out, out_ld, out_col = tail
            td = L.BlockTailDesc(2, None, self._pptr(pname + ".gamma"), self._pptr(pname + ".beta"), out.data_ptr(), out_ld, out_col)
            self._call(self.fwd, "cr_block_ln_ffn_fwd_tail", C.byref(bd), C.byref(td))
        if not self.training:
            return

        def factory():
            lst = []
            dy, dx = self._grad_of(y), self._grad_of(x)
            do = self.buf(pfx + "do", D)
            dqkv = self.buf(pfx + "dqkv", D, rows=3 * M)
            stats = self.vec(pfx + "stats", H * B * T * 4)
            G = self._gptr
            bbd = L.BlockBwdDesc(L.BlockDesc.from_buffer_copy(bd), dy.data_ptr(), do.data_ptr(), dqkv.data_ptr(), dx.data_ptr(),
                                 self._acc(id(dx)), G(pfx + "ln1.gamma"), G(pfx + "ln1.beta"), G(pfx + "wqkv"), G(pfx + "bqkv"),
                                 G(pfx + "ln2.gamma"), G(pfx + "ln2.beta"), G(pfx + "w1"), G(pfx + "b1"), G(pfx + "w2"), G(pfx + "b2"),
                                 self.Gs.shape[1], self.n_slabs)
            abd = L.AttnBwdDesc(L.AttnDesc.from_buffer_copy(ad), do.data_ptr(), D, dqkv.data_ptr(), dqkv.data_ptr() + MD4,
                                dqkv.data_ptr() + 2 * MD4, D, stats.data_ptr())
            if one_pass:
                delta = self.vec("attn_delta", M)
                dq_part = self.buf("attn_dq_part", D)
                bbd.attn_delta, bbd.dq_part = delta.data_ptr(), dq_part.data_ptr()
                abd.delta, abd.dQ_part = delta.data_ptr(), dq_part.data_ptr()
            elif bf and H == 1:
                delta = self.vec("attn_delta", M)
                bbd.attn_delta = delta.data_ptr()
                abd.delta = delta.data_ptr()
            prec = ATTN_PRECISIONS[self.attn_precision]
            rows_bf = bool(self.fuse_stack_bwd and bf and not one_pass and L.lib.cr_stack_bwd_supported(C.byref(bbd), B, T, prec))
            if (rows_bf and self.fuse_block_bwd and (H == 1 or (H == 2 and D == 64))
                    and L.lib.cr_stack_block_bwd_supported(C.byref(bbd), C.byref(abd.f), B, T, prec)):
                dx2 = self.buf(pfx + "dx2", D)
                dy2 = self._second_grad(y)
                ext = L.BlockBwd1Ext(dy2.data_ptr() if dy2 is not None else None, dx2.data_ptr(), None, None)
                nd = None
                if self._lnf_fused(y):
                    _, pname, lo, lo_ld, lo_col = self._lnf_intent[y.data_ptr()]
                    dlo = self._grad_of(lo)
                    nd = L.LnBwdDesc(y.data_ptr(), D, self._pptr(pname + ".gamma"), dlo.data_ptr() + 4 * lo_col, lo_ld, None, D, 0,
                                     self._gptr(pname + ".gamma"), self._gptr(pname + ".beta"), self.Gs.shape[1], self.n_slabs, M, D, 1e-8)
                    assert id(dy) not in self._grad_written and dy2 is None, "the final LayerNorm must be the only consumer of the stack's output"
                    dlo2 = self._second_grad(lo)
                    if dlo2 is not None:
                        assert dlo2.shape == dlo.shape
                        ext.lnf_dy2 = dlo2.data_ptr() + 4 * lo_col
                    self._keep.append(nd)
                    self._block_slab_range(pname + ".gamma", pname + ".beta")
                sc = None
                rec = self._scatter_recipe.get(x.data_ptr())
                if rec is not None and not bbd.dx_accumulate:
                    self._scatter_claimed.add(x.data_ptr())
                    sc = rec[0](True) if rec[4] else rec[0]()
                    if rec[2]:
                        self._block_slab_range(rec[3], rec[3], 2 * min(self.B, self.n_slabs))
                    if sc.d_addend:
                        dadd2 = self.buf(pfx + "dadd2", D)
                        ext.d_addend2 = dadd2.data_ptr()
                        self._grad2[rec[1].data_ptr()] = dadd2
                        self._grad2_bufs[rec[1].data_ptr()] = (rec[1], dadd2)
                    if rec[4]:
                        if sc.d_addend:
                            self._tg_rows = (self._grad_of(rec[1]), dadd2, D, rec[5])
                        else:
                            self._tg_rows = (dx, dx2, D, rec[5])
                    self._keep.append(sc)
                else:
                    self._grad2[x.data_ptr()] = dx2
                    self._grad2_bufs[x.data_ptr()] = (x, dx2)
                self._keep.append(ext)
                self._block_slab_range(pfx + "ln1.gamma", pfx + "b2")
                self._call(lst, "cr_stack_block_bwd", C.byref(bbd), C.byref(abd.f), C.byref(ext), C.byref(nd) if nd is not None else None,
                           C.byref(sc) if sc is not None else None, B, T, prec)
                return lst
            lst += self._fold_pairs()
            two_heads = (rows_bf and H == 2 and D == 64 and T <= 256 and os.environ.get("CASTREC_BF_TWO_KERNELS") is None
                         and os.environ.get("CASTREC_NO_HEAD_DELTA") != "1")
            if two_heads:
                delta = self.vec("attn_delta_heads", H * M)
                bbd.attn_delta = delta.data_ptr()
                abd.delta = delta.data_ptr()
                nd = None
                if self._lnf_fused(y):
                    _, pname, lo, lo_ld, lo_col = self._lnf_intent[y.data_ptr()]
                    dlo = self._grad_of(lo)
                    nd = L.LnBwdDesc(y.data_ptr(), D, self._pptr(pname + ".gamma"), dlo.data_ptr() + 4 * lo_col, lo_ld, None, D, 0,
                                     self._gptr(pname + ".gamma"), self._gptr(pname + ".beta"), self.Gs.shape[1], self.n_slabs, M, D, 1e-8)
                    assert id(dy) not in self._grad_written, "the final LayerNorm must be the only consumer of the stack's output"
                    self._keep.append(nd)
                self._call(lst, "cr_stack_ffn_bwd_heads", C.byref(bbd), C.byref(nd) if nd is not None else None, B, T, H, prec)
            elif rows_bf and self._lnf_fused(y):
                _, pname, lo, lo_ld, lo_col = self._lnf_intent[y.data_ptr()]
                dlo = self._grad_of(lo)
                nd = L.LnBwdDesc(y.data_ptr(), D, self._pptr(pname + ".gamma"), dlo.data_ptr() + 4 * lo_col, lo_ld, None, D, 0,
                                 self._gptr(pname + ".gamma"), self._gptr(pname + ".beta"), self.Gs.shape[1], self.n_slabs, M, D, 1e-8)
                assert id(dy) not in self._grad_written, "the final LayerNorm must be the only consumer of the stack's output"
                self._call(lst, "cr_stack_ffn_bwd_ln", C.byref(bbd), C.byref(nd), B, T, prec)
            elif rows_bf:
                self._call(lst, "cr_stack_ffn_bwd", C.byref(bbd), B, T, prec)
            else:
                assert not self._lnf_fused(y), "final LayerNorm backward was left to a kernel that does not take it"
                self._call(lst, "cr_block_ln_ffn_bwd", C.byref(bbd))
            self._call(lst, "cr_attn_bwd", C.byref(abd))
            recipe = self._scatter_recipe.get(x.data_ptr())
            if recipe is not None and recipe[4]:
                recipe = None
            if recipe is not None and not recipe[2] and not bbd.dx_accumulate:
                self._scatter_claimed.add(x.data_ptr())
                if rows_bf:
                    self._call(lst, "cr_stack_qkv_bwd_scatter", C.byref(bbd), C.byref(recipe[0]()), B, T, prec)
                else:
                    self._call(lst, "cr_block_ln_qkv_bwd_scatter", C.byref(bbd), C.byref(recipe[0]()))
            elif rows_bf:
                self._call(lst, "cr_stack_qkv_bwd", C.byref(bbd), B, T, prec)
            else:
                self._call(lst, "cr_block_ln_qkv_bwd", C.byref(bbd))
            return lst
        factory.pair_aware = True
        self._bwd_factories.append(factory)

    def _block_slab_range(self, first, last, count=None):
        a = self.layout.entries[first][0] - self.layout.n_table
        off, shape, _, _ = self.layout.entries[last]
        self._block_bwd_ranges.append((a, off + int(np.prod(shape)) - self.layout.n_table, min(self.B, self.n_slabs) if count is None else count))

    def _stack_kernel_fits(self, nblocks, want_attn):
        heads_ok = self.H == 1 or (self.H == 2 and self.D == 64)
        if not (self.fused and self.fuse_stack and nblocks >= 1 and not want_attn and heads_ok and 8 <= self.D <= 64):
            return False
        if self.attn_precision == "f32" or self.T > 256:
            return False
        T16, split = (self.T + 15) // 16 * 16, self.attn_precision == "bf16x3"
        lds = T16 * 64 * 2 * (4 if split else 2) + 3 * 4096 * 2 * (2 if split else 1) + 11 * 64 * 4 + T16 * 4
        if T16 > 208 and (split or self.H != 1):
            return False
        return lds <= 160 * 1024

    def op_stack(self, x, prefix, nblocks, out, out_ld, out_col, want_attn=False):
        wide_tails = (not self.fused and self.fuse_wide and self.attn_precision != "f32" and self.D == 128
                      and os.environ.get("CASTREC_WIDE_NO_TAILS") != "1")
        tails = (self.fused or wide_tails) and self.fuse_tails and nblocks > 0
        stack = self._stack_kernel_fits(nblocks, want_attn)
        emb = None
        if stack and x.data_ptr() in self._pending_embed:
            emb = self._pending_embed.pop(x.data_ptr())
        if nblocks == 0 and x.data_ptr() in self._pending_embed:
            self._call(self.fwd, "cr_embed_fwd", C.byref(self._pending_embed.pop(x.data_ptr())))
        ys = [self.buf("%s.%d.y" % (prefix, i), self.D) for i in range(nblocks)]
        cur = x
        collect = [] if stack else None
        for i in range(nblocks):
            nxt = ys[i]
            aw = None
            if want_attn and i == nblocks - 1:
                self.attn_weights = torch.zeros(self.H * self.B, self.T, self.T, dtype=torch.float32, device=self.dev)
                aw = self.attn_weights
            tail = None
            if tails:
                tail = ("next", "%s.%d." % (prefix, i + 1), ys[i + 1]) if i + 1 < nblocks else ("lnf", prefix + ".lnf", out, out_ld, out_col)
            self.op_block(cur, nxt, "%s.%d." % (prefix, i), attn_out=aw, skip_qkv=tails and i > 0, tail=tail, collect=collect)
            cur = nxt
        if stack:
            for i0 in range(0, nblocks, 4):
                part = collect[i0:i0 + 4]
                bds = (L.BlockDesc * len(part))(*[c[0] for c in part])
                ads = (L.AttnDesc * len(part))(*[c[1] for c in part])
                fin = i0 + 4 >= nblocks
                sd = L.StackDesc(len(part), C.cast(bds, C.POINTER(L.BlockDesc)), C.cast(ads, C.POINTER(L.AttnDesc)),
                                 self._pptr(prefix + ".lnf.gamma") if fin else None, self._pptr(prefix + ".lnf.beta") if fin else None,
                                 out.data_ptr() if fin else None, out_ld, out_col,
                                 C.pointer(emb) if (emb is not None and i0 == 0) else None)
                self._keep.append(emb)
                if not L.lib.cr_stack_fwd_supported(C.byref(sd)):
                    raise RuntimeError("cr_stack_fwd does not take the stack %s it was sized for" % prefix)
                self._keep.append((bds, ads))
                self._call(self.fwd, "cr_stack_fwd", C.byref(sd))
        if (stack and self.training and self.fuse_stack_bwd and self.D <= 64 and self.T <= 224
                and os.environ.get("CASTREC_NO_LNF_FUSION") != "1"):
            self._lnf_intent[cur.data_ptr()] = (out.data_ptr() + 4 * out_col, prefix + ".lnf", out, out_ld, out_col)
        self.op_layernorm(cur, out, out_ld, out_col, prefix + ".lnf", skip_fwd=tails or stack)

    def op_head(self, seq_emb):
        M, D = self.M, self.D
        self.seq_emb = seq_emb
        if not self.training:
            return
        if self.loss in SOFTMAX_LOSSES:
            ds = self._grad_of(seq_emb)
            self._grad_written.add(id(ds))
            prec = L.PREC_BF16 if self.attn_precision == "bf16" else L.PREC_BF16X3
            row, pos, neg, V = seq_emb.data_ptr(), self.ids["pos"].data_ptr(), self.ids["neg"].data_ptr(), self.itemnum + 1
            tail = (ds.data_ptr(), ds.shape[1], self._gptr("item_emb"), None, self._ce_ws.data_ptr(), self._ce_ws.numel())
            if self.loss == "ce":
                op = "cr_softmax_ce"
                d = L.SoftmaxCeDesc(row, seq_emb.shape[1], self._pptr("item_emb"), pos, neg, M, D, V, prec, self.state.data_ptr(), *tail)
            elif self.loss == "gbce":
                op = "cr_gbce"
                d = L.GbceDesc(row, seq_emb.shape[1], self._pptr("item_emb"), pos, neg, M, D, V, self.ce_negatives, prec, self.gbce_beta,
                               None, self.seed & 0xFFFFFFFF, self.state.data_ptr() + 16, self.samples.data_ptr(), self.state.data_ptr(),
                               *tail)
            else:
                op = "cr_sampled_ce"
                pop = self.ce_proposal == "popularity"
                d = L.SampledCeDesc(row, seq_emb.shape[1], self._pptr("item_emb"), pos, neg, M, D, V, self.ce_negatives, prec, None,
                                    self.seed & 0xFFFFFFFF, self.state.data_ptr() + 16, self.samples.data_ptr(), self.state.data_ptr(),
                                    *tail, self.item_cdf.data_ptr() if pop else None, self.item_logq.data_ptr() if pop else None)
            self._call(self.fwd, op, C.byref(d))
            return
        rec = self._ln_recipe.get(seq_emb.data_ptr()) if self.fuse_head_ln else None
        if rec is not None:
            x, pname = rec
            dx = self._grad_of(x)
            assert self._acc(id(dx)) == 0
            self._ln_claimed.add(seq_emb.data_ptr())
            d = L.HeadDesc(seq_emb.data_ptr(), seq_emb.shape[1], self._pptr("item_emb"), self.ids["pos"].data_ptr(),
                           self.ids["neg"].data_ptr(), M, D, self.itemnum + 1, self.state.data_ptr(), None, 0,
                           None if self.use_index else self._gptr("item_emb"), None, None, self._head_coef())
            n = L.LnBwdDesc(x.data_ptr(), D, self._pptr(pname + ".gamma"), None, 0, dx.data_ptr(), D, 0,
                            self._gptr(pname + ".gamma"), self._gptr(pname + ".beta"), self.Gs.shape[1], self.n_slabs, M, D, 1e-8)
            last = self.fwd[-1] if self.fwd else None
            if (self.use_index and last is not None and last[0] == "cr_stack_fwd" and os.environ.get("CASTREC_NO_HEAD_FUSION") != "1"
                    and last[2][0]._obj.out == seq_emb.data_ptr()
                    and L.lib.cr_stack_fwd_head_supported(last[2][0], C.byref(d), C.byref(n))):
                self._keep += [d, n]
                self.fwd[-1] = ("cr_stack_fwd_head", L.lib.cr_stack_fwd_head, (last[2][0], C.byref(d), C.byref(n)))
                self._block_slab_range(pname + ".gamma", pname + ".beta", 2 * self.B)
                return
            self._call(self.fwd, "cr_head_fwd_bwd_ln", C.byref(d), C.byref(n))
            return
        ds = self._grad_of(seq_emb)
        self._grad_written.add(id(ds))
        d = L.HeadDesc(seq_emb.data_ptr(), seq_emb.shape[1], self._pptr("item_emb"), self.ids["pos"].data_ptr(),
                       self.ids["neg"].data_ptr(), M, D, self.itemnum + 1, self.state.data_ptr(), ds.data_ptr(), ds.shape[1],
                       None if self.use_index else self._gptr("item_emb"), None, None, self._head_coef())
        self._call(self.fwd, "cr_head_fwd_bwd", C.byref(d))

    def _head_coef(self):
        if not self.use_index:
            return None
        return self.vec("head.coef", 2 * self.M).data_ptr()

    def _build(self):
        m, D, T, L_ = self.model, self.D, self.T, self.hp.num_blocks
        sq = math.sqrt(D)
        st = model_structure(m, self.hp)
        wa_ctx = self.want_attn and m in ("cast_1", "cast_2", "cast_3", "cast_4", "cast_5", "cast_6")
        wa_trunk = self.want_attn and not wa_ctx

        def ctx_stack(table, ids_key, prefix, out, out_ld, out_col, want=False):
            e = self.buf(prefix + ".emb", D)
            self.op_embed(ids_key, table, e, D, 0, sq, small=True, into_stack=True)
            self.op_stack(e, prefix, st["ctx"][prefix], out, out_ld, out_col, want_attn=want)

        if m in ("sasrec", "sasrec_static"):
            x = self.buf("x0", D)
            self.op_embed("seq", "item_emb", x, D, 0, sq, pos="learned" if m == "sasrec" else "static",
                          drop_site="emb", mask=True, into_stack=True)
            s = self.buf("seq_emb", D)
            self.op_stack(x, "trunk", L_, s, D, 0, want_attn=wa_trunk)
        elif m == "cast_1":
            tseq = self.buf("tseq", D)
            ctx_stack("time_emb", "time", "ctx_time", tseq, D, 0, want=wa_ctx)
            x = self.buf("x0", D)
            self.op_embed("seq", "item_emb", x, D, 0, sq, pos="static", addend=(tseq, self._grad_of(tseq)),
                          drop_site="emb", mask=True, into_stack=True)
            s = self.buf("seq_emb", D)
            self.op_stack(x, "trunk", L_, s, D, 0)
        elif m in ("cast_2", "cast_3", "cast_4", "cast_7", "cast_8", "cast_9"):
            k = st["mlp"]
            c = self.buf("concat", k * D)
            if m == "cast_2":
                ctx_stack("time_emb", "time", "ctx_time", c, k * D, D, want=wa_ctx)
                self.op_embed("seq", "item_emb", c, k * D, 0, sq, pos="static", mask=True)
                self.op_dropout_inplace(c, 2 * D, "concat1")
            elif m == "cast_3":
                tseq = self.buf("tseq", D)
                ctx_stack("time_emb", "time", "ctx_time", tseq, D, 0, want=wa_ctx)
                self.op_embed("hours", "hours_emb", c, k * D, D, sq, small=True)
                self.op_embed("days", "days_emb", c, k * D, 2 * D, sq, small=True)
                self.op_embed("seq", "item_emb", c, k * D, 0, sq, pos="static", addend=(tseq, self._grad_of(tseq)),
                              mask=True)
                self.op_dropout_inplace(c, 3 * D, "concat1")
            elif m == "cast_4":
                ctx_stack("time_emb", "time", "ctx_time", c, k * D, D, want=wa_ctx)
                self.op_embed("seq", "item_emb", c, k * D, 0, sq, pos="static", mask=True)
                self.op_dropout_inplace(c, 2 * D, "concat1")
                self.op_embed("hours", "hours_emb", c, k * D, 2 * D, sq, small=True)
                self.op_embed("days", "days_emb", c, k * D, 3 * D, sq, small=True)
                self.op_dropout_inplace(c, 4 * D, "concat2")
            elif m in ("cast_7", "cast_8"):
                if m == "cast_7":
                    self.op_embed("hours", "hours_emb", c, k * D, D, sq, small=True)
                    self.op_embed("days", "days_emb", c, k * D, 2 * D, sq, small=True)
                else:
                    ctx_stack("hours_emb", "hours", "ctx_hours", c, k * D, D)
                    ctx_stack("days_emb", "days", "ctx_days", c, k * D, 2 * D)
                self.op_embed("seq", "item_emb", c, k * D, 0, sq, pos="static", mask=True)
                self.op_dropout_inplace(c, 3 * D, "concat1")
            else:
                ctx_stack("hours_emb", "hours", "ctx_hours", c, k * D, 2 * D)
                ctx_stack("days_emb", "days", "ctx_days", c, k * D, 3 * D)
                ctx_stack("time_emb", "time", "ctx_time", c, k * D, D)
                self.op_embed("seq", "item_emb", c, k * D, 0, sq, pos="learned")
                self.op_dropout_inplace(c, 4 * D, "concat1")
            x = self.buf("x0", D)
            self.op_mlp(c, x, k, mask_out=(m == "cast_9"))
            s = self.buf("seq_emb", D)
            self.op_stack(x, "trunk", L_, s, D, 0, want_attn=wa_trunk)
        elif m in ("cast_5", "cast_6"):
            k = st["mlp"]
            c = self.buf("concat", k * D)
            x = self.buf("x0", D)
            if m == "cast_5":
                tseq = self.buf("tseq", D)
                ctx_stack("time_emb", "time", "ctx_time", tseq, D, 0, want=wa_ctx)
                self.op_embed("seq", "item_emb", x, D, 0, sq, pos="static", addend=(tseq, self._grad_of(tseq)),
                              into_stack=True)
                self.op_stack(x, "trunk", L_, c, k * D, 0)
                self.op_embed("hours", "hours_emb", c, k * D, D, sq, small=True)
                self.op_embed("days", "days_emb", c, k * D, 2 * D, sq, small=True)
                self.op_dropout_inplace(c, 3 * D, "concat1")
            else:
                self.op_embed("seq", "item_emb", x, D, 0, sq, pos="static", into_stack=True)
                self.op_stack(x, "trunk", L_, c, k * D, 0)
                ctx_stack("time_emb", "time", "ctx_time", c, k * D, D, want=wa_ctx)
                self.op_dropout_inplace(c, 2 * D, "concat1")
                self.op_embed("hours", "hours_emb", c, k * D, 2 * D, sq, small=True)
                self.op_embed("days", "days_emb", c, k * D, 3 * D, sq, small=True)
                self.op_dropout_inplace(c, 4 * D, "concat2")
            s = self.buf("seq_emb", D)
            self.op_mlp(c, s, k)
        self.op_head(s)

    def _finalize(self):
        if self.training:
            for fac in reversed(self._bwd_factories):
                lst = fac()
                if lst and self._grad2 and not getattr(fac, "pair_aware", False):
                    self.bwd += self._fold_pairs()
                self.bwd += lst
            assert not self._grad2, "a gradient partial was left without a consumer"
            self.bwd_table_done = 0
            for i, (name, _, a) in enumerate(self.bwd):
                sc = a[0] if name == "cr_embed_bwd" else (a[4] if name == "cr_stack_block_bwd" else (a[1] if name.endswith("_scatter") else None))
                if sc is not None and sc._obj.n_slabs == 0:
                    self.bwd_table_done = i + 1
            lay = self.layout
            snap, tsnap = self.state.data_ptr() + 4 * 8, self.state.data_ptr() + 4 * 11
            l2 = float(self.hp.l2_emb)
            n_l2 = lay.n_l2 if l2 != 0.0 else 0
            lazy = (None, 0, 0, 0, None)
            if self.lazy_adam:
                self.lazy_flags = torch.zeros(self.itemnum + 1, dtype=torch.int32, device=self.dev)
                world = max(1, self.batch_global // self.B)
                self.lazy_ids = self.ids_all[:3].reshape(-1) if world == 1 else torch.zeros(world * 3 * self.M, dtype=torch.int32, device=self.dev)
                lazy = (self.lazy_ids.data_ptr(), self.lazy_ids.numel(), self.itemnum + 1, self.D, self.lazy_flags.data_ptr())
            counts = None
            per = np.full(lay.n_dense, self.n_slabs, np.int32)
            if self.n_wslabs < self.n_slabs:
                for a, b in self._wgrad_ranges:
                    per[a:b] = self.n_wslabs
            for a, b, c in self._block_bwd_ranges:
                per[a:b] = c
            if lay.n_dense and int(per.min()) < self.n_slabs:
                nb = (lay.n_dense + 255) // 256
                pad = np.zeros(nb * 256, np.int32)
                pad[:lay.n_dense] = per
                cnt = pad.reshape(nb, 256).max(1).astype(np.int32)
                self.slab_counts = torch.from_numpy(cnt).to(self.dev)
                counts = self.slab_counts.data_ptr()
            ad = L.AdamDesc(self.P.data_ptr(), self.Mom.data_ptr(), self.Vel.data_ptr(), self.Gt.data_ptr(), self.Gs.data_ptr(),
                            lay.n_table, lay.n_dense, self.n_slabs, float(self.hp.lr), 0.9, 0.98, 1e-8, self.state.data_ptr(),
                            snap, tsnap, l2, n_l2, *lazy, counts)
            self._tgd, self._tgrad = None, None
            if self.use_index:
                assert self._tg_rows is not None, "occurrence index: no gradient-row buffer for the item table's seq lookup"
                rows, rows2, ld_rows, scale = self._tg_rows
                se = self.seq_emb
                self._tgd = L.TgradDesc(self.batch_buf.data_ptr() + 4 * self.index_off, None, 0, 0, 0, self.state.data_ptr() + 4 * 4,
                                        self.index_lay, rows.data_ptr(), rows2.data_ptr() if rows2 is not None else None, ld_rows, scale,
                                        se.data_ptr(), se.shape[1], self._head_coef(), self.D, self._tg_part.data_ptr(), self._tg_tickets.data_ptr())
                ad.tg = C.pointer(self._tgd)
                self._tgrad = ("cr_table_grad", L.lib.cr_table_grad, (C.byref(self._tgd), self.Gt.data_ptr()))
            self._adam = ("cr_adam_step", L.lib.cr_adam_step, (C.byref(ad),))
            ad1 = L.AdamDesc(self.P.data_ptr(), self.Mom.data_ptr(), self.Vel.data_ptr(), self.Gt.data_ptr(),
                             self.Gflat.data_ptr() + 4 * lay.n_table, lay.n_table, lay.n_dense, 1, float(self.hp.lr), 0.9, 0.98,
                             1e-8, self.state.data_ptr(), self.Gflat.data_ptr() + 4 * lay.n_total, tsnap, l2, n_l2, *lazy, None)
            self._adam_flat = ("cr_adam_step", L.lib.cr_adam_step, (C.byref(ad1),))
            self._reduce = ("cr_reduce_slabs", L.lib.cr_reduce_slabs,
                            (self.Gs.data_ptr(), self.n_slabs, lay.n_dense, self.Gflat.data_ptr() + 4 * lay.n_table,
                             self.state.data_ptr(), self.Gflat.data_ptr() + 4 * lay.n_total, counts))
            self._l2 = ("cr_l2_penalty", L.lib.cr_l2_penalty, (self.P.data_ptr(), n_l2, 0.5 * l2, self.state.data_ptr())) if n_l2 else None
            self._keep += [ad, ad1]

    def set_batch(self, seq, pos=None, neg=None, time=None, hours=None, days=None):
        limits = dict(seq=self.itemnum, pos=self.itemnum, neg=self.itemnum, time=self.hp.max_bins, hours=24, days=7)
        used = {"seq", "pos", "neg"} | ({"time"} if "time_emb" in self.layout.entries else set()) \
            | ({"hours", "days"} if "hours_emb" in self.layout.entries else set())
        for k, a in (("seq", seq), ("pos", pos), ("neg", neg), ("time", time), ("hours", hours), ("days", days)):
            if a is None:
                continue
            if self._check_ids and k in used and not isinstance(a, torch.Tensor):
                a = np.asarray(a)
                if a.size and (int(a.min()) < 0 or int(a.max()) > limits[k]):
                    raise ValueError("%s ids outside [0, %d] (min %d, max %d): the lookup table has %d rows"
                                     % (k, limits[k], int(a.min()), int(a.max()), limits[k] + 1))
            t = a if isinstance(a, torch.Tensor) else torch.from_numpy(np.ascontiguousarray(np.asarray(a), dtype=np.int32))
            if self.use_index:
                i = self.ID_KEYS.index(k)
                self._host_slot[i * self.M:(i + 1) * self.M] = t.reshape(-1).to(torch.int32).cpu().numpy()
            else:
                self.ids[k].copy_(t.reshape(-1).to(torch.int32), non_blocking=True)
        if self.use_index:
            used = self._build_index(self._host_slot)
            self.batch_buf[:used].copy_(torch.from_numpy(self._host_slot[:used]))

    def _build_index(self, host_slot):
        M = self.M
        base = host_slot.ctypes.data
        L.check(L.lib.cr_index_build(self._ixb, base, base + 4 * M, base + 8 * M, base + 4 * self.index_off), "cr_index_build")
        return self.index_off + int(host_slot[self.index_off + 4])

    def pack_slot(self, seq, pos, neg, time=None, hours=None, days=None, out=None):
        host = np.zeros(self.slot_words, np.int32) if out is None else out
        for i, a in enumerate((seq, pos, neg, time, hours, days)):
            if a is None:
                host[i * self.M:(i + 1) * self.M] = 0
            else:
                host[i * self.M:(i + 1) * self.M] = np.asarray(a).reshape(-1)
        if self.use_index:
            self._build_index(host)
        return host

    def load_slot(self, slot):
        self.batch_buf.copy_(slot.reshape(-1))

    def set_step(self, k=1):
        self.state[:4].zero_()
        self.state[8:].zero_()
        self.state[4:5].view(torch.int32)[0] = k
        if getattr(self, "_feed_ring", None) is not None:
            if self._feed_have:
                raise RuntimeError("set_step(): %d fed batches are waiting (their ring slots follow the step number)" % self._feed_have)
            self._feed_next, self._feed_started, self._feed_first = int(k), False, int(k)
            torch.cuda.synchronize()
            self._feed_done.clear()
        if getattr(self, "_tg_tickets", None) is not None:
            self._tg_tickets.zero_()
        if getattr(self, "lazy_flags", None) is not None:
            self.lazy_flags.zero_()

    def set_item_weights(self, w):
        if getattr(self, "ce_proposal", "uniform") != "popularity":
            raise RuntimeError("set_item_weights(): this engine was not built with ce_proposal='popularity'")
        from .proposal import build_proposal
        cdf, logq = build_proposal(w, self.itemnum + 1)
        self.item_cdf.copy_(torch.from_numpy(cdf.view(np.int32)))
        self.item_logq.copy_(torch.from_numpy(logq))
        self._have_item_weights = True

    def _need_item_weights(self):
        if self.ce_proposal == "popularity" and not self._have_item_weights:
            raise RuntimeError("ce_proposal='popularity': call set_item_weights() before the first training step")

    def step_number(self):
        return int(self.state[4:5].view(torch.int32)[0])

    def _run(self, lst, stream):
        for name, fn, args in lst:
            rc = fn(*args, stream)
            if rc != 0:
                raise RuntimeError("castrec %s failed (%d): %s" % (name, rc, L.lib.cr_last_error().decode()))

    def launch_step(self, apply=True, between=None, capturing=False):
        s = torch.cuda.current_stream().cuda_stream
        if self.training and not capturing:
            self._need_item_weights()
        self._run(self.fwd, s)
        if self.training:
            self._run(self.bwd, s)
            if between is not None:
                between()
            if apply:
                self._run(([self._l2] if self._l2 else []) + [self._adam], s)
                if self._id_ring is not None and self.lazy_adam:
                    self._run([self._ring_next], s)

    def use_id_ring(self, ring):
        ads = [self._adam[2][0]._obj, self._adam_flat[2][0]._obj]
        if ring is None:
            self._id_ring = None
            for ad in ads:
                ad.ids_ring, ad.ids_ring_slots, ad.ids_slot_elems, ad.ids_dst, ad.ids_copy_elems = None, 0, 0, None, 0
            if self._tgd is not None:
                self._tgd.ring, self._tgd.ring_slots, self._tgd.slot_words, self._tgd.index_off = None, 0, 0, 0
            return
        assert ring.dtype == torch.int32 and ring.is_cuda and ring.is_contiguous(), ring.shape
        assert int(np.prod(ring.shape[1:])) == self.slot_words, \
            "ring slots of %s words, the engine's slots have %d (pack_slot: 6 x %d ids%s)" % (tuple(ring.shape[1:]), self.slot_words, self.M, " + the occurrence index" if self.use_index else "")
        self._id_ring = ring
        if self.lazy_adam:
            self._ring_next = ("cr_ids_ring_next", L.lib.cr_ids_ring_next,
                               (ring.data_ptr(), int(ring.shape[0]), 6 * self.M, self.ids_all.data_ptr(), self.state.data_ptr() + 4 * 11))
        else:
            for ad in ads:
                ad.ids_ring, ad.ids_ring_slots, ad.ids_slot_elems, ad.ids_dst = ring.data_ptr(), int(ring.shape[0]), self.slot_words, self.ids_all.data_ptr()
                ad.ids_copy_elems = self.ids_words
            if self._tgd is not None:
                self._tgd.ring, self._tgd.ring_slots, self._tgd.slot_words, self._tgd.index_off = ring.data_ptr(), int(ring.shape[0]), self.slot_words, self.index_off

    def enable_feed(self, n_slots=8, steps_per_graph=1):
        assert self.training and n_slots >= 4
        self._feed_every = 4 if n_slots >= 8 else 1
        self._feed_ring = torch.zeros(n_slots, self.slot_words, dtype=torch.int32, device=self.dev)
        self._feed_host = torch.zeros(n_slots, self.slot_words, dtype=torch.int32).pin_memory()
        self._feed_np = self._feed_host.numpy()
        self._feed_stream = torch.cuda.Stream()
        self._feed_h2d = [None] * n_slots
        self._feed_done = {}
        recapture = self.graph is not None
        self.use_id_ring(self._feed_ring)
        if recapture:
            assert steps_per_graph == 1 or n_slots >= 2 * steps_per_graph + 4, "ring too small for %d steps per launch" % steps_per_graph
            self.capture(n_steps=steps_per_graph if not self.lazy_adam else 1)
        self._feed_next, self._feed_have, self._feed_started = self.step_number(), 0, False
        self._feed_first = self._feed_next
        used = {"seq", "pos", "neg"} | ({"time"} if "time_emb" in self.layout.entries else set()) \
            | ({"hours", "days"} if "hours_emb" in self.layout.entries else set())
        limits = dict(seq=self.itemnum, pos=self.itemnum, neg=self.itemnum, time=self.hp.max_bins, hours=24, days=7)
        self._feed_limits = [(i, k, limits[k]) for i, k in enumerate(self.ID_KEYS) if k in used]

    def feed(self, seq, pos, neg, time=None, hours=None, days=None):
        n = self._feed_ring.shape[0]
        if self._feed_have > min(n - self._feed_every, n - 2):
            raise RuntimeError("feed(): %d batches are waiting already (ring of %d slots)" % (self._feed_have, n))
        k = self._feed_next
        slot = k % n
        if self._feed_h2d[slot] is not None:
            self._feed_h2d[slot].synchronize()
        host = self._feed_np[slot]
        hid = host[:self.ids_words].reshape(6, self.M)
        for i, a in enumerate((seq, pos, neg, time, hours, days)):
            if a is None:
                hid[i] = 0
            else:
                hid[i] = np.asarray(a).reshape(-1)
# ... 24 lines not shown
            raise RuntimeError("train_fed(): no batch has been fed")
        self._need_item_weights()
        n = self._feed_ring.shape[0]
        k = self._feed_next - self._feed_have
        G = self.graph_steps if (getattr(self, "graph_multi", None) is not None and self.graph is not None) else 1
        if self._feed_have < G or (max_steps is not None and max_steps < G):
            G = 1
        cur = torch.cuda.current_stream()
        if not self._feed_started:
            self._feed_h2d[k % n].synchronize()
            self.ids_all.copy_(self._feed_ring[k % n][:self.ids_words].view(6, self.M))
        for j in range(1, min(G, self._feed_have - 1) + 1):
            self._feed_h2d[(k + j) % n].synchronize()
        self._feed_started = self._feed_have >= G + 1
        if G > 1:
            self.graph_multi.launch()
        elif self.graph is not None:
            self.graph.launch()
        else:
            self.launch_step()
        last = k + G - 1
        marks = [j for j in range(k, last + 1) if j % self._feed_every == 0]
        if G > 1 and last not in marks:
            marks.append(last)
        if marks:
            ev = torch.cuda.Event()
            ev.record(cur)
            for j in marks:
                self._feed_done[j] = ev
            for old in [j for j in self._feed_done if j < last - n]:
                del self._feed_done[old]
        self._feed_have -= G
        return G

    def launch_backward_to_flat(self):
        s = torch.cuda.current_stream().cuda_stream
        self._run(self.fwd, s)
        self._run(self.bwd, s)
        self._run(([self._tgrad] if self._tgrad else []) + [self._reduce], s)

    def launch_adam_from_flat(self):
        self._run(([self._l2] if self._l2 else []) + [self._adam_flat], torch.cuda.current_stream().cuda_stream)

    def capture_dp_phases(self):
        s0 = torch.cuda.current_stream()
        side = torch.cuda.Stream()
        side.wait_stream(s0)
        k = self.bwd_table_done
        progs = [self.fwd + self.bwd[:k] + ([self._tgrad] if self._tgrad else []), self.bwd[k:] + [self._reduce],
                 ([self._l2] if self._l2 else []) + [self._adam_flat]]
        graphs = []
        with torch.cuda.stream(side):
            for prog in progs:
                g = O.Graph()
                g.begin()
                self._run(prog, torch.cuda.current_stream().cuda_stream)
                g.end()
                graphs.append(g)
        s0.wait_stream(side)
        self.dp_graphs, self.dp_progs, self._graph_stream = graphs, progs, side
        return graphs

    def capture(self, dp=False, n_steps=1):
        side = torch.cuda.Stream()
        side.wait_stream(torch.cuda.current_stream())
        g = O.Graph()
        with torch.cuda.stream(side):
            g.begin()
            if dp:
                self.launch_backward_to_flat()
            else:
                self.launch_step(capturing=True)
            g.end()
        self.graph_multi, self.graph_steps = None, 1
        if n_steps > 1:
            assert not dp and self.training and self._id_ring is not None and not self.lazy_adam, "several steps per graph need the id ring (use_id_ring / enable_feed)"
            gm = O.Graph()
            with torch.cuda.stream(side):
                gm.begin()
                for _ in range(n_steps):
                    self.launch_step(capturing=True)
                gm.end()
            self.graph_multi, self.graph_steps = gm, int(n_steps)
        torch.cuda.current_stream().wait_stream(side)
        self.graph, self._graph_stream = g, side
        return g

    def train_step(self, seq, pos, neg, time=None, hours=None, days=None):
        self.set_batch(seq, pos, neg, time, hours, days)
        if self.graph is not None:
            self._need_item_weights()
            self.graph.launch()
        else:
            self.launch_step()

    def loss_auc(self):
        s = self.state.cpu()
        return float(s[5]), float(s[6])

    def forward_eval(self, seq, time=None, hours=None, days=None):
        assert not self.training
        self.set_batch(seq, None, None, time, hours, days)
        self.launch_step()

    def test_logits(self, cand):
        out = torch.empty(self.B, cand.shape[1], dtype=torch.float32, device=self.dev)
        O.test_logits(self.seq_emb, self.seq_emb.shape[1], self.p("item_emb"), cand, self.B, self.T, self.D, out)
        return out

    def topk(self, k, excl_off=None, excl_ids=None, targets=None, index=None):
        B, V, D = self.B, self.itemnum + 1, self.D
        need = O.topk_workspace_bytes(B, V, D, int(k))
        ws = getattr(self, "_topk_ws", None)
        if ws is None or ws.numel() < need:
            ws = self._topk_ws = torch.empty(need, dtype=torch.uint8, device=self.dev)
        if excl_ids is not None and not torch.is_tensor(excl_ids):
            excl_ids = torch.from_numpy(np.ascontiguousarray(excl_ids, np.int32))
        if excl_ids is not None:
            excl_ids = excl_ids.to(self.dev, torch.int32).contiguous()
            if excl_ids.numel() == 0:
                excl_ids = None
                excl_off = None
        if targets is not None:
            targets = torch.as_tensor(np.asarray(targets, np.int32) if not torch.is_tensor(targets) else targets).to(self.dev, torch.int32).contiguous()
        ids = torch.empty(B, int(k), dtype=torch.int32, device=self.dev)
        scores = torch.empty(B, int(k), dtype=torch.float32, device=self.dev)
        rank = torch.empty(B, dtype=torch.int32, device=self.dev) if targets is not None else None
        prec = L.PREC_BF16 if self.attn_precision == "bf16" else L.PREC_BF16X3
        se = self.seq_emb
        ld = se.shape[1]
        query = se[self.T - 1:]
        if index is not None:
            if (index.V, index.D) != (V, D):
                raise ValueError("index of a [%d, %d] table, the engine's item table is [%d, %d]" % (index.V, index.D, V, D))
            O.score_topk(query, self.T * ld, (V, D), B, int(k), prec, excl_off, excl_ids, targets, ws, ids, scores, rank,
                         index=index.blob, index_precision=index.prec)
            return ids, scores, rank
        O.score_topk(query, self.T * ld, self.p("item_emb"), B, int(k), prec, excl_off, excl_ids, targets, ws, ids, scores, rank)
        return ids, scores, rank

    def get_params(self):
        return {n: self.layout.view(self.P, n).detach().clone() for n in self.layout.logical_names()}

    def load_params(self, d):
        for n in self.layout.logical_names():
            self.layout.view(self.P, n).copy_(torch.tensor(np.asarray(d[n]), dtype=torch.float32).to(self.dev))

    def grads(self):
        n = float(self.state[2])
        if self._tgrad is not None:
            self.Gt.zero_()
            self._run([self._tgrad], torch.cuda.current_stream().cuda_stream)
            torch.cuda.synchronize()
        flat = torch.cat([self.Gt, self.Gs.sum(0)[:self.layout.n_dense]]) / max(n, 1.0)
        return {k: self.layout.view(flat, k).clone() for k in self.layout.logical_names()}

    def n_launches(self):
        return len(self.fwd) + len(self.bwd) + (1 if self.training else 0) + (1 if self.training and self._l2 else 0)

    def n_kernel_launches(self):
        n = 0
        pair_max = int(os.environ.get("CASTREC_STACK_PAIR_MAX_B", 160))
        for name, _, args in self.fwd + self.bwd:
            if name in ("cr_stack_fwd", "cr_stack_fwd_head"):
                sd = args[0]._obj
                n += sd.n_blocks if (self.B <= pair_max and self.T > 16) else 1
            elif name == "cr_stack_block_bwd":
                per = min(self.B, self.n_slabs)
                n += -(-self.B // per)
            else:
                n += 1
        return n + (1 if self.training else 0) + (1 if self.training and self._l2 else 0)
```

### context-aware-sequential-recommendation_amd/lib.py

```python
import ctypes as C
import os

import torch

from . import PKG_DIR

LIB_PATH = os.path.join(PKG_DIR, "libcastrec_tl.so" if os.environ.get("CASTREC_TIMELINE") == "1" else "libcastrec.so")
if os.environ.get("CASTREC_LIB"):
    LIB_PATH = os.path.abspath(os.environ["CASTREC_LIB"])
if not os.path.exists(LIB_PATH):
    raise ImportError("castrec_amd: native library %s not found -- build it with "
                      "`python -m castrec_amd.build` (needs hipcc, gfx950). There is no CPU fallback." % LIB_PATH)
_lib = C.CDLL(LIB_PATH)

c_f = C.c_float
c_i = C.c_int
c_u32 = C.c_uint32
c_p = C.c_void_p

CR_MAX_BATCH = 4
CR_STATE_FLOATS = 16
CR_SCE_MAX_SAMPLES = 16384
CR_SCE_SITE = 0x5CE00000
CR_GBCE_SITE = 0x6BCE0000
PREC_F32, PREC_BF16X3, PREC_BF16 = 0, 1, 2
ELT_COPY, ELT_ADD, ELT_DROPOUT, ELT_RELU_BWD, ELT_ROWMASK, ELT_GRADPREP = 0, 1, 2, 3, 4, 5


class Rng(C.Structure):
    _fields_ = [("rate", c_f), ("site", c_u32), ("seed", c_u32), ("step", c_p), ("row_offset", c_u32)]


class EmbedDesc(C.Structure):
    _fields_ = [("ids", c_p), ("table", c_p), ("M", c_i), ("T", c_i), ("D", c_i), ("V", c_i),
                ("zero_pad", c_i), ("scale", c_f), ("pos_table", c_p), ("addend", c_p), ("ld_add", c_i),
                ("drop", Rng), ("mask_ids", c_p), ("out", c_p), ("ld_out", c_i), ("col_off", c_i)]


class EmbedBwdDesc(C.Structure):
    _fields_ = [("f", EmbedDesc), ("table_grad", c_p), ("pos_grad", c_p), ("d_addend", c_p),
                ("slab_stride", c_i), ("n_slabs", c_i), ("out2", c_p)]


class LnDesc(C.Structure):
    _fields_ = [("x", c_p), ("ldx", c_i), ("gamma", c_p), ("beta", c_p), ("y", c_p), ("ldy", c_i),
                ("M", c_i), ("D", c_i), ("eps", c_f), ("x_nonzero", c_p), ("y_nonzero", c_p)]


class LnBwdDesc(C.Structure):
    _fields_ = [("x", c_p), ("ldx", c_i), ("gamma", c_p), ("dy", c_p), ("lddy", c_i), ("dx", c_p), ("lddx", c_i),
                ("accumulate", c_i), ("dgamma", c_p), ("dbeta", c_p), ("slab_stride", c_i), ("n_slabs", c_i),
                ("M", c_i), ("D", c_i), ("eps", c_f)]


class GemmDesc(C.Structure):
    _fields_ = [("A", c_p), ("lda", c_i), ("B", c_p), ("ldb", c_i), ("bias", c_p), ("C", c_p), ("ldc", c_i),
                ("M", c_i), ("N", c_i), ("K", c_i), ("trans_b", c_i), ("relu", c_i), ("drop", Rng),
                ("residual", c_p), ("ldr", c_i), ("mask_ids", c_p), ("accumulate", c_i), ("precision", c_i)]


class WgradDesc(C.Structure):
    _fields_ = [("A", c_p), ("lda", c_i), ("G", c_p), ("ldg", c_i), ("dW", c_p), ("ldw", c_i), ("db", c_p),
                ("M", c_i), ("N", c_i), ("K", c_i), ("precision", c_i)]


class EltDesc(C.Structure):
    _fields_ = [("op", c_i), ("x", c_p), ("ldx", c_i), ("aux", c_p), ("ldaux", c_i), ("y", c_p), ("ldy", c_i),
                ("M", c_i), ("N", c_i), ("drop", Rng), ("mask_ids", c_p), ("accumulate", c_i)]


class AttnDesc(C.Structure):
    _fields_ = [("Q", c_p), ("K", c_p), ("V", c_p), ("ld", c_i), ("k_valid", c_p), ("q_valid", c_p),
                ("residual", c_p), ("ldr", c_i), ("dead_ids", c_p), ("out", c_p), ("ldo", c_i),
                ("attn_weights", c_p), ("B", c_i), ("T", c_i), ("H", c_i), ("d", c_i), ("drop", Rng),
                ("batch_global", c_i), ("row_stats", c_p), ("precision", c_i)]


class AttnBwdDesc(C.Structure):
    _fields_ = [("f", AttnDesc), ("dout", c_p), ("lddo", c_i), ("dQ", c_p), ("dK", c_p), ("dV", c_p),
                ("ldg", c_i), ("stats", c_p), ("delta", c_p), ("dQ_part", c_p)]


class BlockDesc(C.Structure):
    _fields_ = [("M", c_i), ("D", c_i), ("ln1_g", c_p), ("ln1_b", c_p), ("wqkv", c_p), ("bqkv", c_p), ("ln2_g", c_p),
                ("ln2_b", c_p), ("w1", c_p), ("b1", c_p), ("w2", c_p), ("b2", c_p), ("x", c_p), ("q_in", c_p), ("qkv", c_p),
                ("k_valid", c_p), ("q_valid", c_p), ("o", c_p), ("f_in", c_p), ("hid", c_p), ("y", c_p), ("mask_ids", c_p),
                ("drop_ffn1", Rng), ("drop_ffn2", Rng)]


class BlockBwdDesc(C.Structure):
    _fields_ = [("f", BlockDesc), ("dy", c_p), ("d_o", c_p), ("dqkv", c_p), ("dx", c_p), ("dx_accumulate", c_i),
                ("g_ln1_g", c_p), ("g_ln1_b", c_p), ("g_wqkv", c_p), ("g_bqkv", c_p), ("g_ln2_g", c_p), ("g_ln2_b", c_p),
                ("g_w1", c_p), ("g_b1", c_p), ("g_w2", c_p), ("g_b2", c_p), ("slab_stride", c_i), ("n_slabs", c_i),
                ("attn_delta", c_p), ("dq_part", c_p)]


class BlockBwd1Ext(C.Structure):
    _fields_ = [("dy2", c_p), ("dx2", c_p), ("lnf_dy2", c_p), ("d_addend2", c_p)]


class BlockTailDesc(C.Structure):
    _fields_ = [("kind", c_i), ("next", C.POINTER(BlockDesc)), ("lnf_gamma", c_p), ("lnf_beta", c_p), ("out", c_p),
                ("ld_out", c_i), ("col_out", c_i)]


class StackDesc(C.Structure):
    _fields_ = [("n_blocks", c_i), ("blocks", C.POINTER(BlockDesc)), ("attn", C.POINTER(AttnDesc)), ("lnf_gamma", c_p),
                ("lnf_beta", c_p), ("out", c_p), ("ld_out", c_i), ("col_out", c_i), ("embed", C.POINTER(EmbedDesc))]


class HeadDesc(C.Structure):
    _fields_ = [("seq_emb", c_p), ("ld", c_i), ("table", c_p), ("pos", c_p), ("neg", c_p),
                ("M", c_i), ("D", c_i), ("V", c_i), ("state", c_p), ("d_seq_emb", c_p), ("ldd", c_i),
                ("table_grad", c_p), ("pos_logits", c_p), ("neg_logits", c_p), ("coef_out", c_p)]


class IndexLayout(C.Structure):
    _fields_ = [("M", c_i), ("V", c_i), ("T_pos", c_i), ("ng", c_i), ("ent", c_i), ("cap_blocks", c_i), ("cap_occ", c_i), ("bitmap_words", c_i),
                ("off_recs", C.c_int64), ("total_words", C.c_int64)]


class TgradDesc(C.Structure):
    _fields_ = [("index", c_p), ("ring", c_p), ("ring_slots", c_i), ("slot_words", C.c_int64), ("index_off", C.c_int64), ("step", c_p),
                ("lay", IndexLayout), ("rows", c_p), ("rows2", c_p), ("ld_rows", c_i), ("scale", c_f), ("seq_emb", c_p), ("ld_emb", c_i),
                ("coef", c_p), ("D", c_i), ("part_rows", c_p), ("tickets", c_p)]


class AdamDesc(C.Structure):
    _fields_ = [("p", c_p), ("m", c_p), ("v", c_p), ("table_grad", c_p), ("dense_slabs", c_p),
                ("n_table", C.c_int64), ("n_dense", c_i), ("n_slabs", c_i), ("lr", c_f), ("beta1", c_f),
                ("beta2", c_f), ("eps", c_f), ("state", c_p), ("stats", c_p), ("step_snapshot", c_p), ("l2", c_f), ("n_l2", C.c_int64),
                ("lazy_ids", c_p), ("n_lazy_ids", c_i), ("lazy_rows", c_i), ("lazy_D", c_i), ("lazy_flags", c_p), ("slab_counts", c_p),
                ("ids_ring", c_p), ("ids_ring_slots", c_i), ("ids_slot_elems", C.c_int64), ("ids_dst", c_p),
                ("ids_copy_elems", C.c_int64), ("tg", C.POINTER(TgradDesc))]


CR_TOPK_MAX = 128


class TopkDesc(C.Structure):
    _fields_ = [("query", c_p), ("ld", c_i), ("table", c_p), ("V", c_i), ("D", c_i), ("B", c_i), ("K", c_i), ("precision", c_i),
                ("excl_off", c_p), ("excl_ids", c_p), ("targets", c_p), ("top_ids", c_p), ("top_scores", c_p), ("rank", c_p),
                ("workspace", c_p), ("workspace_bytes", C.c_size_t),
                ("index", c_p), ("index_bytes", C.c_size_t), ("index_precision", c_i)]


class SoftmaxCeDesc(C.Structure):
    _fields_ = [("seq_emb", c_p), ("ld", c_i), ("table", c_p), ("pos", c_p), ("neg", c_p), ("M", c_i), ("D", c_i), ("V", c_i),
                ("precision", c_i), ("state", c_p), ("d_seq_emb", c_p), ("ldd", c_i), ("table_grad", c_p), ("lse_out", c_p),
                ("workspace", c_p), ("workspace_bytes", C.c_size_t)]


class SampledCeDesc(C.Structure):
    _fields_ = [("seq_emb", c_p), ("ld", c_i), ("table", c_p), ("pos", c_p), ("neg", c_p), ("M", c_i), ("D", c_i), ("V", c_i),
                ("N", c_i), ("precision", c_i), ("samples", c_p), ("seed", C.c_uint32), ("step", c_p), ("samples_out", c_p),
                ("state", c_p), ("d_seq_emb", c_p), ("ldd", c_i), ("table_grad", c_p), ("lse_out", c_p), ("workspace", c_p),
                ("workspace_bytes", C.c_size_t), ("cdf", c_p), ("logq", c_p)]


class GbceDesc(C.Structure):
    _fields_ = [("seq_emb", c_p), ("ld", c_i), ("table", c_p), ("pos", c_p), ("neg", c_p), ("M", c_i), ("D", c_i), ("V", c_i),
                ("N", c_i), ("precision", c_i), ("beta", c_f), ("samples", c_p), ("seed", C.c_uint32), ("step", c_p),
                ("samples_out", c_p), ("state", c_p), ("d_seq_emb", c_p), ("ldd", c_i), ("table_grad", c_p), ("loss_out", c_p),
                ("workspace", c_p), ("workspace_bytes", C.c_size_t)]


def _sig(name, restype, argtypes):
    f = getattr(_lib, name)
    f.restype = restype
    f.argtypes = argtypes
    return f


_sig("cr_version", c_i, [])
_sig("cr_last_error", C.c_char_p, [])
_sig("cr_step_begin", c_i, [c_p, c_p])
_sig("cr_ids_ring_next", c_i, [c_p, c_i, C.c_int64, c_p, c_p, c_p])
_sig("cr_embed_fwd", c_i, [C.POINTER(EmbedDesc), c_p])
_sig("cr_embed_bwd", c_i, [C.POINTER(EmbedBwdDesc), c_p])
_sig("cr_layernorm_fwd", c_i, [C.POINTER(LnDesc), c_p])
_sig("cr_layernorm_bwd", c_i, [C.POINTER(LnBwdDesc), c_p])
_sig("cr_gemm_rows", c_i, [C.POINTER(GemmDesc), c_i, c_p])
_sig("cr_gemm_wgrad", c_i, [C.POINTER(WgradDesc), c_i, c_i, c_i, c_p])
_sig("cr_eltwise", c_i, [C.POINTER(EltDesc), c_p])
_sig("cr_attn_fwd", c_i, [C.POINTER(AttnDesc), c_p])
_sig("cr_attn_bwd", c_i, [C.POINTER(AttnBwdDesc), c_p])
_sig("cr_block_ln_qkv_fwd", c_i, [C.POINTER(BlockDesc), c_p])
_sig("cr_block_ln_qkv_fwd_gather", c_i, [C.POINTER(BlockDesc), C.POINTER(EmbedDesc), c_p])
_sig("cr_block_ln_ffn_fwd", c_i, [C.POINTER(BlockDesc), c_p])
_sig("cr_block_ln_ffn_fwd_tail", c_i, [C.POINTER(BlockDesc), C.POINTER(BlockTailDesc), c_p])
_sig("cr_stack_fwd_supported", c_i, [C.POINTER(StackDesc)])
_sig("cr_stack_fwd", c_i, [C.POINTER(StackDesc), c_p])
_sig("cr_block_ln_ffn_bwd", c_i, [C.POINTER(BlockBwdDesc), c_p])
_sig("cr_block_ln_qkv_bwd", c_i, [C.POINTER(BlockBwdDesc), c_p])
_sig("cr_stack_bwd_supported", c_i, [C.POINTER(BlockBwdDesc), c_i, c_i, c_i])
_sig("cr_stack_ffn_bwd", c_i, [C.POINTER(BlockBwdDesc), c_i, c_i, c_i, c_p])
_sig("cr_stack_ffn_bwd_ln", c_i, [C.POINTER(BlockBwdDesc), C.POINTER(LnBwdDesc), c_i, c_i, c_i, c_p])
_sig("cr_stack_ffn_bwd_heads", c_i, [C.POINTER(BlockBwdDesc), C.POINTER(LnBwdDesc), c_i, c_i, c_i, c_i, c_p])
_sig("cr_stack_qkv_bwd", c_i, [C.POINTER(BlockBwdDesc), c_i, c_i, c_i, c_p])
_sig("cr_stack_qkv_bwd_scatter", c_i, [C.POINTER(BlockBwdDesc), C.POINTER(EmbedBwdDesc), c_i, c_i, c_i, c_p])
_sig("cr_stack_block_bwd_supported", c_i, [C.POINTER(BlockBwdDesc), C.POINTER(AttnDesc), c_i, c_i, c_i])
_sig("cr_stack_block_bwd_deal", c_i, [c_i, c_i, C.POINTER(C.c_uint32)])
_sig("cr_stack_block_bwd", c_i, [C.POINTER(BlockBwdDesc), C.POINTER(AttnDesc), C.POINTER(BlockBwd1Ext), C.POINTER(LnBwdDesc), C.POINTER(EmbedBwdDesc),
                                 c_i, c_i, c_i, c_p])
_sig("cr_block_ln_qkv_bwd_scatter", c_i, [C.POINTER(BlockBwdDesc), C.POINTER(EmbedBwdDesc), c_p])
_sig("cr_wide_supported", c_i, [C.POINTER(BlockDesc), c_i])
_sig("cr_wide_ln_qkv_fwd", c_i, [C.POINTER(BlockDesc), c_i, c_p])
_sig("cr_wide_ln_ffn_fwd", c_i, [C.POINTER(BlockDesc), c_i, c_p])
_sig("cr_wide_ln_ffn_fwd_tail", c_i, [C.POINTER(BlockDesc), C.POINTER(BlockTailDesc), c_i, c_p])
_sig("cr_wide_ln_ffn_bwd", c_i, [C.POINTER(BlockBwdDesc), c_p, c_p, c_i, c_i, c_p])
_sig("cr_wide_ln_qkv_bwd", c_i, [C.POINTER(BlockBwdDesc), c_i, c_p])
_sig("cr_head_fwd_bwd", c_i, [C.POINTER(HeadDesc), c_p])
_sig("cr_head_fwd_bwd_ln", c_i, [C.POINTER(HeadDesc), C.POINTER(LnBwdDesc), c_p])
_sig("cr_stack_fwd_head_supported", c_i, [C.POINTER(StackDesc), C.POINTER(HeadDesc), C.POINTER(LnBwdDesc)])
_sig("cr_stack_fwd_head", c_i, [C.POINTER(StackDesc), C.POINTER(HeadDesc), C.POINTER(LnBwdDesc), c_p])
_sig("cr_test_logits", c_i, [c_p, c_i, c_p, c_p, c_i, c_i, c_i, c_i, c_i, c_p, c_p])
_sig("cr_adam_step", c_i, [C.POINTER(AdamDesc), c_p])
_sig("cr_reduce_slabs", c_i, [c_p, c_i, c_i, c_p, c_p, c_p, c_p, c_p])
_sig("cr_l2_penalty", c_i, [c_p, C.c_int64, c_f, c_p, c_p])
_sig("cr_rows_pack", c_i, [c_p, c_p, c_i, c_i, c_i, c_p, c_p, c_p, c_i, c_p])
_sig("cr_rows_add", c_i, [c_p, c_p, c_i, c_i, c_i, c_p])
_sig("cr_graph_begin", c_i, [c_p])
_sig("cr_graph_end", c_i, [c_p, C.POINTER(c_p)])
_sig("cr_graph_launch", c_i, [c_p, c_p])
_sig("cr_graph_destroy", c_i, [c_p])
_sig("cr_sampler_create", c_p, [c_p, c_p, c_p, c_p, c_i, c_i, c_i, c_i, c_i, c_i, c_i, C.c_double, C.c_double, c_u32, c_i])
_sig("cr_sampler_next", c_i, [c_p] + [c_p] * 8)
_sig("cr_sampler_destroy", None, [c_p])
_sig("cr_tgrad_geometry", c_i, [c_i, C.POINTER(c_i), C.POINTER(c_i)])
_sig("cr_batch_index_layout", c_i, [c_i, c_i, c_i, c_i, c_i, C.POINTER(IndexLayout)])
_sig("cr_index_builder_create", c_p, [c_i, c_i, c_i, c_i, c_i])
_sig("cr_index_build", c_i, [c_p, c_p, c_p, c_p, c_p])
_sig("cr_index_builder_destroy", None, [c_p])
_sig("cr_table_grad", c_i, [C.POINTER(TgradDesc), c_p, c_p])
_sig("cr_score_topk_workspace", C.c_size_t, [c_i, c_i, c_i, c_i])
_sig("cr_score_topk", c_i, [C.POINTER(TopkDesc), c_p])
_sig("cr_topk_index_bytes", C.c_size_t, [c_i, c_i, c_i])
_sig("cr_topk_index_build", c_i, [c_p, c_i, c_i, c_i, c_p, C.c_size_t, c_p])
_sig("cr_softmax_ce_workspace", C.c_size_t, [c_i, c_i, c_i])
_sig("cr_softmax_ce", c_i, [C.POINTER(SoftmaxCeDesc), c_p])
_sig("cr_sampled_ce_workspace", C.c_size_t, [c_i, c_i, c_i])
_sig("cr_sampled_ce", c_i, [C.POINTER(SampledCeDesc), c_p])
_sig("cr_gbce_workspace", C.c_size_t, [c_i, c_i, c_i])
_sig("cr_gbce", c_i, [C.POINTER(GbceDesc), c_p])

EXPORTS = ["cr_version", "cr_last_error", "cr_step_begin", "cr_ids_ring_next", "cr_embed_fwd", "cr_embed_bwd", "cr_layernorm_fwd",
           "cr_layernorm_bwd", "cr_gemm_rows", "cr_gemm_wgrad", "cr_eltwise", "cr_attn_fwd", "cr_attn_bwd",
           "cr_block_ln_qkv_fwd", "cr_block_ln_qkv_fwd_gather", "cr_block_ln_ffn_fwd", "cr_block_ln_ffn_fwd_tail", "cr_stack_fwd_supported", "cr_stack_fwd", "cr_block_ln_ffn_bwd", "cr_block_ln_qkv_bwd", "cr_stack_bwd_supported", "cr_stack_ffn_bwd", "cr_stack_ffn_bwd_ln", "cr_stack_ffn_bwd_heads", "cr_stack_qkv_bwd", "cr_stack_qkv_bwd_scatter", "cr_stack_block_bwd_supported", "cr_stack_block_bwd", "cr_stack_block_bwd_deal", "cr_rows_pack", "cr_rows_add", "cr_block_ln_qkv_bwd_scatter",
           "cr_wide_supported", "cr_wide_ln_qkv_fwd", "cr_wide_ln_ffn_fwd", "cr_wide_ln_ffn_fwd_tail", "cr_wide_ln_ffn_bwd", "cr_wide_ln_qkv_bwd",
           "cr_head_fwd_bwd", "cr_head_fwd_bwd_ln", "cr_stack_fwd_head_supported", "cr_stack_fwd_head", "cr_test_logits", "cr_adam_step", "cr_reduce_slabs", "cr_l2_penalty", "cr_graph_begin", "cr_graph_end", "cr_graph_launch",
           "cr_graph_destroy", "cr_sampler_create", "cr_sampler_next", "cr_sampler_destroy",
           "cr_tgrad_geometry", "cr_batch_index_layout", "cr_index_builder_create", "cr_index_build", "cr_index_builder_destroy", "cr_table_grad",
           "cr_score_topk_workspace", "cr_score_topk", "cr_topk_index_bytes", "cr_topk_index_build", "cr_softmax_ce_workspace", "cr_softmax_ce",
           "cr_sampled_ce_workspace", "cr_sampled_ce", "cr_gbce_workspace", "cr_gbce"]

lib = _lib


def check(rc, what=""):
    if rc != 0:
        raise RuntimeError("castrec %s failed (%d): %s" % (what, rc, _lib.cr_last_error().decode()))


def call(name, *args):
    check(getattr(_lib, name)(*args), name)
```

### include/castrec.h

```cpp
#ifndef CASTREC_H
#define CASTREC_H

#include <stddef.h>
#include <stdint.h>

#ifdef __cplusplus
extern "C" {
#endif

#define CR_OK 0
#define CR_ERR_INVALID (-1)
#define CR_ERR_UNSUPPORTED (-2)
#define CR_ERR_HIP (-3)

#define CR_MAX_BATCH 4
#define CR_STATE_FLOATS 16

int cr_version(void);
const char* cr_last_error(void);

typedef struct {
    float rate;
    uint32_t site;
    uint32_t seed;
// ... 48 lines not shown
    const float* dy; int lddy;
    float* dx; int lddx;
    int accumulate;
    float* dgamma; float* dbeta;
    int slab_stride, n_slabs;
    int M, D;
    float eps;
} cr_ln_bwd_desc;
int cr_layernorm_bwd(const cr_ln_bwd_desc* d, void* stream);

#define CR_PREC_F32 0
#define CR_PREC_BF16X3 1
#define CR_PREC_BF16 2

typedef struct {
    const float* A; int lda;
    const float* B; int ldb;
    const float* bias;
    float* C; int ldc;
    int M, N, K;
    int trans_b;
    int relu;
    cr_rng drop;
    const float* residual; int ldr;
    const int32_t* mask_ids;
    int accumulate;
    int precision;
} cr_gemm_desc;
int cr_gemm_rows(const cr_gemm_desc* d, int n_problems, void* stream);

typedef struct {
    const float* A; int lda;
    const float* G; int ldg;
    float* dW; int ldw;
    float* db;
    int M, N, K;
    int precision;
} cr_wgrad_desc;
int cr_gemm_wgrad(const cr_wgrad_desc* d, int n_problems, int slab_stride, int n_slabs, void* stream);

#define CR_ELT_COPY 0
#define CR_ELT_ADD 1
#define CR_ELT_DROPOUT 2
#define CR_ELT_RELU_BWD 3
#define CR_ELT_ROWMASK 4
#define CR_ELT_GRADPREP 5
typedef struct {
    int op;
    const float* x; int ldx;
    const float* aux; int ldaux;
    float* y; int ldy;
    int M, N;
    cr_rng drop;
    const int32_t* mask_ids;
    int accumulate;
} cr_elt_desc;
int cr_eltwise(const cr_elt_desc* d, void* stream);


typedef struct {
    const float* Q; const float* K; const float* V; int ld;
    const float* k_valid;
    const float* q_valid;
    const float* residual; int ldr;
    const int32_t* dead_ids;
    float* out; int ldo;
    float* attn_weights;
    int B, T, H, d;
    cr_rng drop;
    int batch_global;
    float* row_stats;
    int precision;
} cr_attn_desc;
int cr_attn_fwd(const cr_attn_desc* d, void* stream);

typedef struct {
    cr_attn_desc f;
    const float* dout; int lddo;
    float* dQ; float* dK; float* dV; int ldg;
    float* stats;
    const float* delta;
    float* dQ_part;
} cr_attn_bwd_desc;
int cr_attn_bwd(const cr_attn_bwd_desc* d, void* stream);

typedef struct {
    int M, D;
    const float* ln1_g; const float* ln1_b;
    const float* wqkv; const float* bqkv;
    const float* ln2_g; const float* ln2_b;
    const float* w1; const float* b1; const float* w2; const float* b2;
    const float* x;
    float* q_in; float* qkv;
    float* k_valid; float* q_valid;
    float* o;
    float* f_in; float* hid; float* y;
    const int32_t* mask_ids;
    cr_rng drop_ffn1, drop_ffn2;
} cr_block_desc;
int cr_block_ln_qkv_fwd(const cr_block_desc* d, void* stream);
int cr_block_ln_ffn_fwd(const cr_block_desc* d, void* stream);

int cr_block_ln_qkv_fwd_gather(const cr_block_desc* d, const cr_embed_desc* e, void* stream);

typedef struct {
    int kind;
    const cr_block_desc* next;
    const float* lnf_gamma; const float* lnf_beta; float* out; int ld_out, col_out;
} cr_block_tail_desc;
int cr_block_ln_ffn_fwd_tail(const cr_block_desc* d, const cr_block_tail_desc* t, void* stream);

#define CR_STACK_MAX_BLOCKS 4
typedef struct {
    int n_blocks;
    const cr_block_desc* blocks;
    const cr_attn_desc* attn;
    const float* lnf_gamma; const float* lnf_beta; float* out; int ld_out, col_out;
    const cr_embed_desc* embed;
} cr_stack_desc;
int cr_stack_fwd_supported(const cr_stack_desc* d);
int cr_stack_fwd(const cr_stack_desc* d, void* stream);

typedef struct {
    cr_block_desc f;
    const float* dy;
    float* d_o;
    const float* dqkv;
    float* dx; int dx_accumulate;
    float* g_ln1_g; float* g_ln1_b; float* g_wqkv; float* g_bqkv;
    float* g_ln2_g; float* g_ln2_b; float* g_w1; float* g_b1; float* g_w2; float* g_b2;
    int slab_stride, n_slabs;
    float* attn_delta;
    const float* dq_part;
} cr_block_bwd_desc;
int cr_block_ln_ffn_bwd(const cr_block_bwd_desc* d, void* stream);
int cr_block_ln_qkv_bwd(const cr_block_bwd_desc* d, void* stream);

int cr_stack_bwd_supported(const cr_block_bwd_desc* d, int B, int T, int precision);
int cr_stack_ffn_bwd(const cr_block_bwd_desc* d, int B, int T, int precision, void* stream);
int cr_stack_ffn_bwd_ln(const cr_block_bwd_desc* d, const cr_ln_bwd_desc* n, int B, int T, int precision, void* stream);
int cr_stack_ffn_bwd_heads(const cr_block_bwd_desc* d, const cr_ln_bwd_desc* n, int B, int T, int heads, int precision, void* stream);
int cr_stack_qkv_bwd(const cr_block_bwd_desc* d, int B, int T, int precision, void* stream);
int cr_stack_qkv_bwd_scatter(const cr_block_bwd_desc* d, const cr_embed_bwd_desc* sc, int B, int T, int precision, void* stream);

typedef struct {
    const float* dy2;
    float* dx2;
    const float* lnf_dy2;
    float* d_addend2;
} cr_block_bwd1_ext;
int cr_stack_block_bwd_supported(const cr_block_bwd_desc* d, const cr_attn_desc* ad, int B, int T, int precision);
int cr_stack_block_bwd(const cr_block_bwd_desc* d, const cr_attn_desc* ad, const cr_block_bwd1_ext* x, const cr_ln_bwd_desc* lnf,
                       const cr_embed_bwd_desc* sc, int B, int T, int precision, void* stream);
int cr_stack_block_bwd_deal(int tiles, int query_pass, uint32_t* pk);

int cr_wide_supported(const cr_block_desc* d, int precision);
int cr_wide_ln_qkv_fwd(const cr_block_desc* d, int precision, void* stream);
int cr_wide_ln_ffn_fwd(const cr_block_desc* d, int precision, void* stream);
int cr_wide_ln_ffn_fwd_tail(const cr_block_desc* d, const cr_block_tail_desc* t, int precision, void* stream);
int cr_wide_ln_ffn_bwd(const cr_block_bwd_desc* d, float* g2, float* g1, int heads, int precision, void* stream);
int cr_wide_ln_qkv_bwd(const cr_block_bwd_desc* d, int precision, void* stream);

int cr_block_ln_qkv_bwd_scatter(const cr_block_bwd_desc* bd, const cr_embed_bwd_desc* sc, void* stream);

typedef struct {
    const float* seq_emb; int ld;
    const float* table;
    const int32_t* pos; const int32_t* neg;
    int M, D, V;
    float* state;
    float* d_seq_emb; int ldd;
    float* table_grad;
    float* pos_logits; float* neg_logits;
    float* coef_out;
} cr_head_desc;
int cr_head_fwd_bwd(const cr_head_desc* d, void* stream);

int cr_head_fwd_bwd_ln(const cr_head_desc* d, const cr_ln_bwd_desc* n, void* stream);

int cr_stack_fwd_head_supported(const cr_stack_desc* d, const cr_head_desc* h, const cr_ln_bwd_desc* n);
int cr_stack_fwd_head(const cr_stack_desc* d, const cr_head_desc* h, const cr_ln_bwd_desc* n, void* stream);

int cr_test_logits(const float* seq_emb, int ld, const float* table, const int32_t* cand,
                   int B, int T, int D, int V, int n_cand, float* logits, void* stream);

#define CR_TOPK_MAX 128
typedef struct cr_topk_desc cr_topk_desc;
struct cr_topk_desc {
    const float* query; int ld;
    const float* table;
    int V, D, B, K;
    int precision;
    const int64_t* excl_off;
    const int32_t* excl_ids;
    const int32_t* targets;
    int32_t* top_ids;
    float* top_scores;
    int32_t* rank;
    void* workspace;
    size_t workspace_bytes;
    const void* index;
    size_t index_bytes;
    int index_precision;
};
size_t cr_score_topk_workspace(int B, int V, int D, int K);
int cr_score_topk(const cr_topk_desc* d, void* stream);

size_t cr_topk_index_bytes(int V, int D, int precision);
int cr_topk_index_build(const float* table, int V, int D, int precision, void* index, size_t index_bytes, void* stream);

typedef struct cr_softmax_ce_desc cr_softmax_ce_desc;
struct cr_softmax_ce_desc {
    const float* seq_emb; int ld;
    const float* table;
    const int32_t* pos;
    const int32_t* neg;
    int M, D, V;
    int precision;
    float* state;
    float* d_seq_emb; int ldd;
    float* table_grad;
    float* lse_out;
    void* workspace;
    size_t workspace_bytes;
};
size_t cr_softmax_ce_workspace(int M, int V, int D);
int cr_softmax_ce(const cr_softmax_ce_desc* d, void* stream);

#define CR_SCE_MAX_SAMPLES 16384
#define CR_SCE_SITE 0x5CE00000u
typedef struct cr_sampled_ce_desc cr_sampled_ce_desc;
struct cr_sampled_ce_desc {
    const float* seq_emb; int ld;
    const float* table;
    const int32_t* pos;
    const int32_t* neg;
    int M, D, V, N;
    int precision;
    const int32_t* samples;
    uint32_t seed;
    const uint32_t* step;
    int32_t* samples_out;
    float* state;
    float* d_seq_emb; int ldd;
    float* table_grad;
    float* lse_out;
    void* workspace;
    size_t workspace_bytes;
    const uint32_t* cdf;
    const float* logq;
};
size_t cr_sampled_ce_workspace(int M, int N, int D);
int cr_sampled_ce(const cr_sampled_ce_desc* d, void* stream);

#define CR_GBCE_SITE 0x6BCE0000u
typedef struct cr_gbce_desc cr_gbce_desc;
struct cr_gbce_desc {
    const float* seq_emb; int ld;
    const float* table;
    const int32_t* pos;
    const int32_t* neg;
    int M, D, V, N;
    int precision;
    float beta;
    const int32_t* samples;
    uint32_t seed;
    const uint32_t* step;
    int32_t* samples_out;
    float* state;
    float* d_seq_emb; int ldd;
    float* table_grad;
    float* loss_out;
    void* workspace;
    size_t workspace_bytes;
};
size_t cr_gbce_workspace(int M, int N, int D);
int cr_gbce(const cr_gbce_desc* d, void* stream);

#define CR_INDEX_MAGIC 0x43524959
typedef struct {
    int M, V, T_pos;
    int ng, ent;
    int cap_blocks, cap_occ, bitmap_words;
    int64_t off_recs, total_words;
} cr_index_layout;
int cr_tgrad_geometry(int D, int* ng, int* ent);
int cr_batch_index_layout(int M, int V, int T_pos, int ng, int ent, cr_index_layout* out);
typedef struct cr_index_builder cr_index_builder;
cr_index_builder* cr_index_builder_create(int M, int V, int T_pos, int ng, int ent);
int cr_index_build(cr_index_builder* b, const int32_t* seq, const int32_t* pos, const int32_t* neg, int32_t* out);
void cr_index_builder_destroy(cr_index_builder* b);

typedef struct {
    const int32_t* index;
    const int32_t* ring; int ring_slots; int64_t slot_words, index_off;
    const uint32_t* step;
    cr_index_layout lay;
    const float* rows; const float* rows2; int ld_rows;
    float scale;
    const float* seq_emb; int ld_emb;
    const float* coef;
    int D;
    float* part_rows; uint32_t* tickets;
} cr_tgrad_desc;
int cr_table_grad(const cr_tgrad_desc* d, float* table_grad, void* stream);

// ... 48 lines not shown
```

Before: 413,300 sequences/s.

## Fold finished dense-gradient slab columns inside later block-backward launches

Adds a third grid row (blockIdx.y==2) to the fused block-backward kernel. It sums the per-slab partial gradients of 256-column blocks whose writers have already finished, and writes each result into slab 0. A host-side planner picks which column blocks each launch can fold and sets their slab count to 1. The Adam kernel then reads a single slab for those blocks instead of reducing many. This moves reduction work off the optimizer's critical path into idle workgroups of an earlier launch, at the cost of a bigger grid and extra work competing in that kernel.

```diff
diff --git a/context-aware-sequential-recommendation_amd/build.py b/context-aware-sequential-recommendation_amd/build.py
--- a/context-aware-sequential-recommendation_amd/build.py
+++ b/context-aware-sequential-recommendation_amd/build.py
@@ -150,7 +150,7 @@
     return [f for f in flags if not (f == "-fno-slp-vectorize" and source_name in slp_ok)]
 
 
-HEADERS = [os.path.join(CSRC, h) for h in ("cr_common.hpp", "cr_attn_common.hpp", "cr_bf16.hpp", "cr_rlayout.hpp", "cr_rbwd.hpp")] \
+HEADERS = [os.path.join(CSRC, h) for h in ("cr_common.hpp", "cr_attn_common.hpp", "cr_bf16.hpp", "cr_rlayout.hpp", "cr_rbwd.hpp", "cr_slabsum.hpp")] \
     + [os.path.join(ROOT, "include", "castrec.h")]
 EXTRA_DEPS = {"cr_adam.hip": ["cr_tgrad.hpp"], "cr_tgrad.hip": ["cr_tgrad.hpp"]}
 
diff --git a/context-aware-sequential-recommendation_amd/csrc/cr_adam.hip b/context-aware-sequential-recommendation_amd/csrc/cr_adam.hip
--- a/context-aware-sequential-recommendation_amd/csrc/cr_adam.hip
+++ b/context-aware-sequential-recommendation_amd/csrc/cr_adam.hip
@@ -4,41 +4,9 @@
 
 #include "cr_common.hpp"
 #include "cr_tgrad.hpp"
+#include "cr_slabsum.hpp"
 
 int tg_unit_grid(const cr_tgrad_desc* d);
-
-#define ADAM_COLS 256
-#define ADAM_WAVES 16
-typedef float f4a __attribute__((ext_vector_type(4), aligned(4)));
-__device__ __forceinline__ float slab_sum256(const float* slabs, int n_slabs, int n_dense, int j0, float (*part)[ADAM_COLS]) {
-    const int lane = threadIdx.x & 63, w = threadIdx.x >> 6;
-    const int j = j0 + 4 * lane;
-    f4a acc = (f4a){0.f, 0.f, 0.f, 0.f};
-    if (j + 3 < n_dense) {
-        for (int s0 = w; s0 < n_slabs; s0 += 16 * ADAM_WAVES) {
-            f4a v[16];
-            int cnt = 0;
-#pragma unroll
-            for (int u = 0; u < 16; ++u)
-                if (s0 + ADAM_WAVES * u < n_slabs) { v[u] = *reinterpret_cast<const f4a*>(slabs + (size_t)(s0 + ADAM_WAVES * u) * n_dense + j); cnt = u + 1; }
-#pragma unroll
-            for (int u = 0; u < 16; ++u)
-                if (u < cnt) acc += v[u];
-        }
-    } else {
-        for (int s = w; s < n_slabs; s += ADAM_WAVES)
-            for (int u = 0; u < 4; ++u)
-                if (j + u < n_dense) acc[u] += slabs[(size_t)s * n_dense + j + u];
-    }
-    part[w][4 * lane + 0] = acc.x; part[w][4 * lane + 1] = acc.y; part[w][4 * lane + 2] = acc.z; part[w][4 * lane + 3] = acc.w;
-    __syncthreads();
-    float g = 0.0f;
-    if (threadIdx.x < ADAM_COLS) {
-#pragma unroll
-        for (int k = 0; k < ADAM_WAVES; ++k) g += part[k][threadIdx.x];
-    }
-    return g;
-}
 
 template <bool STREAM, int LPR, int VEC>
 __global__ __launch_bounds__(64 * ADAM_WAVES) void k_adam(cr_adam_desc d, cr_tgrad_desc g, int nb_dense, int nb_lazy, int nb_units, int nb_ring) {
diff --git a/context-aware-sequential-recommendation_amd/csrc/cr_slabsum.hpp b/context-aware-sequential-recommendation_amd/csrc/cr_slabsum.hpp
--- /dev/null
+++ b/context-aware-sequential-recommendation_amd/csrc/cr_slabsum.hpp
@@ -0,0 +1,40 @@
+#pragma once
+
+#define ADAM_COLS 256
+#define ADAM_WAVES 16
+typedef float f4a __attribute__((ext_vector_type(4), aligned(4)));
+
+template <int NW = ADAM_WAVES>
+__device__ __forceinline__ float slab_sum256(const float* slabs, int n_slabs, int n_dense, int j0, float (*part)[ADAM_COLS]) {
+    static_assert(NW > 0 && ADAM_WAVES % NW == 0, "the real waves share the 16 virtual ones evenly");
+    const int lane = threadIdx.x & 63;
+    const int j = j0 + 4 * lane;
+#pragma unroll
+    for (int w = threadIdx.x >> 6; w < ADAM_WAVES; w += NW) {
+        f4a acc = (f4a){0.f, 0.f, 0.f, 0.f};
+        if (j + 3 < n_dense) {
+            for (int s0 = w; s0 < n_slabs; s0 += 16 * ADAM_WAVES) {
+                f4a v[16];
+                int cnt = 0;
+#pragma unroll
+                for (int u = 0; u < 16; ++u)
+                    if (s0 + ADAM_WAVES * u < n_slabs) { v[u] = *reinterpret_cast<const f4a*>(slabs + (size_t)(s0 + ADAM_WAVES * u) * n_dense + j); cnt = u + 1; }
+#pragma unroll
+                for (int u = 0; u < 16; ++u)
+                    if (u < cnt) acc += v[u];
+            }
+        } else {
+            for (int s = w; s < n_slabs; s += ADAM_WAVES)
+                for (int u = 0; u < 4; ++u)
+                    if (j + u < n_dense) acc[u] += slabs[(size_t)s * n_dense + j + u];
+        }
+        part[w][4 * lane + 0] = acc.x; part[w][4 * lane + 1] = acc.y; part[w][4 * lane + 2] = acc.z; part[w][4 * lane + 3] = acc.w;
+    }
+    __syncthreads();
+    float g = 0.0f;
+    if (threadIdx.x < ADAM_COLS) {
+#pragma unroll
+        for (int k = 0; k < ADAM_WAVES; ++k) g += part[k][threadIdx.x];
+    }
+    return g;
+}
diff --git a/context-aware-sequential-recommendation_amd/csrc/cr_stack_bwd1.hip b/context-aware-sequential-recommendation_amd/csrc/cr_stack_bwd1.hip
--- a/context-aware-sequential-recommendation_amd/csrc/cr_stack_bwd1.hip
+++ b/context-aware-sequential-recommendation_amd/csrc/cr_stack_bwd1.hip
@@ -5,6 +5,7 @@
 #include <mutex>
 
 #include "cr_rbwd.hpp"
+#include "cr_slabsum.hpp"
 
 #define B1_DRAIN() asm volatile("s_waitcnt vmcnt(0)" ::: "memory")
 #define B1_NT_WS true
@@ -34,6 +35,13 @@
     float isd, isd_log2e, invT;
     unsigned qpk[8], kpk[8];
     unsigned long long* ts;
+};
+
+#define B1_FOLD_MAX 128
+struct B1Fold {
+    float* slabs;
+    int stride, n;
+    unsigned pk[B1_FOLD_MAX];
 };
 
 __device__ __forceinline__ const B1Args& b1_args_again() {
@@ -1189,9 +1197,25 @@
     B1_TS(5);
 }
 
+__device__ __forceinline__ void b1_fold_role(const B1Fold& f, unsigned char* smem) {
+    float (*part)[ADAM_COLS] = reinterpret_cast<float (*)[ADAM_COLS]>(smem);
+    for (int i = (int)blockIdx.x; i < f.n; i += (int)gridDim.x) {
+        const unsigned e = f.pk[i];
+        const int j0 = (int)(e >> 12) * ADAM_COLS;
+        const float g = slab_sum256<SB_WAVES>(f.slabs, (int)(e & 4095u), f.stride, j0, part);
+        if (threadIdx.x < ADAM_COLS && j0 + (int)threadIdx.x < f.stride) f.slabs[j0 + threadIdx.x] = g;
+        __syncthreads();
+    }
+}
+
 template <bool SPLIT, int DS, int HD>
-__global__ __launch_bounds__(SB_NT) void k_stack_block_bwd(B1Args a) {
+__global__ __launch_bounds__(SB_NT) void k_stack_block_bwd(B1Args a, B1Fold f) {
     extern __shared__ __attribute__((aligned(16))) unsigned char smem_raw[];
+    static_assert(B1Lds<SPLIT>::BYTES >= (int)sizeof(float) * ADAM_WAVES * ADAM_COLS, "the fold role's partials inside the launch's LDS");
+    if (blockIdx.y == 2) {
+        b1_fold_role(f, smem_raw);
+        return;
+    }
     B1_TS(0);
     cr_kernarg_touch<sizeof(B1Args)>();
     B1_TS(15);
@@ -1279,20 +1303,20 @@
 }
 
 template <bool SPLIT, int DS, int HD = 1>
-static int launch_b1(B1Args& a, int nwg, hipStream_t s) {
+static int launch_b1(B1Args& a, const B1Fold& f, int nwg, hipStream_t s) {
     static cr_devmask attr = 0;
     int rc = cr_raise_lds_limit(reinterpret_cast<const void*>(&k_stack_block_bwd<SPLIT, DS, HD>), &attr);
     if (rc) return rc;
     for (int n0 = 0; n0 < a.B; n0 += nwg) {
         a.n0 = n0;
         a.add = n0 > 0;
-        hipLaunchKernelGGL((k_stack_block_bwd<SPLIT, DS, HD>), dim3(a.B - n0 < nwg ? a.B - n0 : nwg, 2), dim3(SB_NT), B1Lds<SPLIT>::BYTES, s, a);
+        hipLaunchKernelGGL((k_stack_block_bwd<SPLIT, DS, HD>), dim3(a.B - n0 < nwg ? a.B - n0 : nwg, f.n > 0 ? 3 : 2), dim3(SB_NT), B1Lds<SPLIT>::BYTES, s, a, f);
     }
     return cr_check_launch("cr_stack_block_bwd");
 }
 
-extern "C" int cr_stack_block_bwd(const cr_block_bwd_desc* bd, const cr_attn_desc* ad, const cr_block_bwd1_ext* x, const cr_ln_bwd_desc* lnf,
-                                  const cr_embed_bwd_desc* sc, int B, int T, int precision, void* stream) {
+static int b1_run(const cr_block_bwd_desc* bd, const cr_attn_desc* ad, const cr_block_bwd1_ext* x, const cr_ln_bwd_desc* lnf,
+                  const cr_embed_bwd_desc* sc, int B, int T, int precision, const B1Fold& fold, void* stream) {
     const char* why = b1_unsupported(bd, ad, B, T, precision);
     CR_REQUIRE(why == nullptr, "cr_stack_block_bwd: unsupported (%s)", why ? why : "");
     CR_REQUIRE(x != nullptr, "cr_stack_block_bwd: NULL extension");
@@ -1356,21 +1380,50 @@
     const bool split = precision == CR_PREC_BF16X3;
     hipStream_t s = cr_stream(stream);
     switch (d->D) {
-    case 64: return split ? launch_b1<true, 64, 2>(a, nwg, s) : launch_b1<false, 64, 2>(a, nwg, s);
+    case 64: return split ? launch_b1<true, 64, 2>(a, fold, nwg, s) : launch_b1<false, 64, 2>(a, fold, nwg, s);
     case 50:
         static const bool no_nk = getenv("CASTREC_B1_NO_NKT") != nullptr;
-        if (a.T == 200 && !no_nk) return split ? launch_b1<true, 50 | (13 << 8) | (200 << 16)>(a, nwg, s) : launch_b1<false, 50 | (13 << 8) | (200 << 16)>(a, nwg, s);
-        return split ? launch_b1<true, 50>(a, nwg, s) : launch_b1<false, 50>(a, nwg, s);
-    case 32: return split ? launch_b1<true, 32>(a, nwg, s) : launch_b1<false, 32>(a, nwg, s);
-    case 40: return split ? launch_b1<true, 40>(a, nwg, s) : launch_b1<false, 40>(a, nwg, s);
-    case 48: return split ? launch_b1<true, 48>(a, nwg, s) : launch_b1<false, 48>(a, nwg, s);
-    case 56: return split ? launch_b1<true, 56>(a, nwg, s) : launch_b1<false, 56>(a, nwg, s);
+        if (a.T == 200 && !no_nk) return split ? launch_b1<true, 50 | (13 << 8) | (200 << 16)>(a, fold, nwg, s) : launch_b1<false, 50 | (13 << 8) | (200 << 16)>(a, fold, nwg, s);
+        return split ? launch_b1<true, 50>(a, fold, nwg, s) : launch_b1<false, 50>(a, fold, nwg, s);
+    case 32: return split ? launch_b1<true, 32>(a, fold, nwg, s) : launch_b1<false, 32>(a, fold, nwg, s);
+    case 40: return split ? launch_b1<true, 40>(a, fold, nwg, s) : launch_b1<false, 40>(a, fold, nwg, s);
+    case 48: return split ? launch_b1<true, 48>(a, fold, nwg, s) : launch_b1<false, 48>(a, fold, nwg, s);
+    case 56: return split ? launch_b1<true, 56>(a, fold, nwg, s) : launch_b1<false, 56>(a, fold, nwg, s);
     default: break;
     }
     switch (d->D / 16) {
-    case 0: return split ? launch_b1<true, -1>(a, nwg, s) : launch_b1<false, -1>(a, nwg, s);
-    case 1: return split ? launch_b1<true, -2>(a, nwg, s) : launch_b1<false, -2>(a, nwg, s);
-    case 2: return split ? launch_b1<true, -3>(a, nwg, s) : launch_b1<false, -3>(a, nwg, s);
-    default: return split ? launch_b1<true, -4>(a, nwg, s) : launch_b1<false, -4>(a, nwg, s);
-    }
-}
+    case 0: return split ? launch_b1<true, -1>(a, fold, nwg, s) : launch_b1<false, -1>(a, fold, nwg, s);
+    case 1: return split ? launch_b1<true, -2>(a, fold, nwg, s) : launch_b1<false, -2>(a, fold, nwg, s);
+    case 2: return split ? launch_b1<true, -3>(a, fold, nwg, s) : launch_b1<false, -3>(a, fold, nwg, s);
+    default: return split ? launch_b1<true, -4>(a, fold, nwg, s) : launch_b1<false, -4>(a, fold, nwg, s);
+    }
+}
+
+extern "C" int cr_stack_block_bwd(const cr_block_bwd_desc* bd, const cr_attn_desc* ad, const cr_block_bwd1_ext* x, const cr_ln_bwd_desc* lnf,
+                                  const cr_embed_bwd_desc* sc, int B, int T, int precision, void* stream) {
+    B1Fold none;
+    memset(static_cast<void*>(&none), 0, sizeof(none));
+    return b1_run(bd, ad, x, lnf, sc, B, T, precision, none, stream);
+}
+
+extern "C" int cr_stack_block_bwd_fold(const cr_block_bwd_desc* bd, const cr_attn_desc* ad, const cr_block_bwd1_ext* x, const cr_ln_bwd_desc* lnf,
+                                       const cr_embed_bwd_desc* sc, int B, int T, int precision, const cr_slab_fold_desc* fold, void* stream) {
+    B1Fold f;
+    memset(static_cast<void*>(&f), 0, sizeof(f));
+    if (fold && fold->n_blocks != 0) {
+        CR_REQUIRE(fold->n_blocks > 0 && fold->n_blocks <= B1_FOLD_MAX, "cr_stack_block_bwd_fold: 0 <= n_blocks <= %d", B1_FOLD_MAX);
+        CR_REQUIRE(fold->slabs && fold->blocks && fold->counts && fold->slab_stride > 0, "cr_stack_block_bwd_fold: slabs / blocks / counts / slab_stride");
+        CR_REQUIRE(bd != nullptr, "cr_stack_block_bwd_fold: NULL description");
+        CR_REQUIRE(B >= 1 && B <= bd->n_slabs, "cr_stack_block_bwd_fold: the fold needs a call of ONE launch (B <= n_slabs)");
+        const int nb = cr_ceil_div(fold->slab_stride, ADAM_COLS);
+        CR_REQUIRE(nb <= (1 << 20), "cr_stack_block_bwd_fold: slab rows of 2^28 floats or more");
+        for (int i = 0; i < fold->n_blocks; ++i) {
+            CR_REQUIRE(fold->blocks[i] >= 0 && fold->blocks[i] < nb, "cr_stack_block_bwd_fold: blocks[%d] = %d outside the %d blocks of the slab row", i, fold->blocks[i], nb);
+            CR_REQUIRE(fold->counts[i] >= 1 && fold->counts[i] <= 4095, "cr_stack_block_bwd_fold: counts[%d] = %d (1 .. 4095 slabs)", i, fold->counts[i]);
+            for (int k = 0; k < i; ++k) CR_REQUIRE(fold->blocks[k] != fold->blocks[i], "cr_stack_block_bwd_fold: block %d listed twice", fold->blocks[i]);
+            f.pk[i] = ((unsigned)fold->blocks[i] << 12) | (unsigned)fold->counts[i];
+        }
+        f.slabs = fold->slabs; f.stride = fold->slab_stride; f.n = fold->n_blocks;
+    }
+    return b1_run(bd, ad, x, lnf, sc, B, T, precision, f, stream);
+}
diff --git a/context-aware-sequential-recommendation_amd/engine.py b/context-aware-sequential-recommendation_amd/engine.py
--- a/context-aware-sequential-recommendation_amd/engine.py
+++ b/context-aware-sequential-recommendation_amd/engine.py
@@ -146,6 +146,35 @@
             elif init == "ones":
                 flat[off:off + size] = 1.0
         return flat
+
+
+SLAB_FOLD_MAX = 128
+
+
+def plan_slab_folds(n_dense, per, known, launches, cap=SLAB_FOLD_MAX):
+    last = np.full(n_dense, -2, np.int64)
+    for a, b, i in known:
+        last[a:b] = np.maximum(last[a:b], i)
+    cnt = slab_block_counts(n_dense, per)
+    plan = {}
+    for k in range(len(cnt)):
+        cols = slice(256 * k, min(256 * k + 256, n_dense))
+        if int(last[cols].min()) == -2 or int(cnt[k]) <= 1:
+            continue
+        w = int(last[cols].max())
+        for i in launches:
+            if i > w and len(plan.get(i, ())) < cap:
+                plan.setdefault(i, []).append((k, int(cnt[k])))
+                cnt[k] = 1
+                break
+    return plan, cnt
+
+
+def slab_block_counts(n_dense, per):
+    nb = (n_dense + 255) // 256
+    pad = np.zeros(nb * 256, np.int32)
+    pad[:n_dense] = per
+    return pad.reshape(nb, 256).max(1).astype(np.int32)
 
 
 class Engine:
@@ -223,6 +252,9 @@
         self._grad2 = {}
         self._grad2_bufs = {}
         self._block_bwd_ranges = []
+        self.slab_fold = os.environ.get("CASTREC_NO_SLAB_FOLD") != "1"
+        self._range_owner = []
+        self.slab_fold_plan = {}
         self.fuse_head_ln = os.environ.get("CASTREC_NO_HEAD_LN") != "1" and self.loss == "bce"
         self._check_ids = os.environ.get("CASTREC_NO_ID_CHECK") != "1"
         self.fused = (4 <= hp.hidden_units <= 64) if fused is None else bool(fused)
@@ -738,6 +770,7 @@
                     and L.lib.cr_stack_block_bwd_supported(C.byref(bbd), C.byref(abd.f), B, T, prec)):
                 dx2 = self.buf(pfx + "dx2", D)
                 dy2 = self._second_grad(y)
+                me = []
                 ext = L.BlockBwd1Ext(dy2.data_ptr() if dy2 is not None else None, dx2.data_ptr(), None, None)
                 nd = None
                 if self._lnf_fused(y):
@@ -751,7 +784,7 @@
                         assert dlo2.shape == dlo.shape
                         ext.lnf_dy2 = dlo2.data_ptr() + 4 * lo_col
                     self._keep.append(nd)
-                    self._block_slab_range(pname + ".gamma", pname + ".beta")
+                    self._block_slab_range(pname + ".gamma", pname + ".beta", owner=me)
                 sc = None
                 rec = self._scatter_recipe.get(x.data_ptr())
                 if rec is not None and not bbd.dx_accumulate:
@@ -774,9 +807,10 @@
                     self._grad2[x.data_ptr()] = dx2
                     self._grad2_bufs[x.data_ptr()] = (x, dx2)
                 self._keep.append(ext)
-                self._block_slab_range(pfx + "ln1.gamma", pfx + "b2")
+                self._block_slab_range(pfx + "ln1.gamma", pfx + "b2", owner=me)
                 self._call(lst, "cr_stack_block_bwd", C.byref(bbd), C.byref(abd.f), C.byref(ext), C.byref(nd) if nd is not None else None,
                            C.byref(sc) if sc is not None else None, B, T, prec)
+                me.append(lst[-1])
                 return lst
             lst += self._fold_pairs()
             two_heads = (rows_bf and H == 2 and D == 64 and T <= 256 and os.environ.get("CASTREC_BF_TWO_KERNELS") is None
@@ -824,10 +858,11 @@
         factory.pair_aware = True
         self._bwd_factories.append(factory)
 
-    def _block_slab_range(self, first, last, count=None):
+    def _block_slab_range(self, first, last, count=None, owner=None):
         a = self.layout.entries[first][0] - self.layout.n_table
         off, shape, _, _ = self.layout.entries[last]
         self._block_bwd_ranges.append((a, off + int(np.prod(shape)) - self.layout.n_table, min(self.B, self.n_slabs) if count is None else count))
+        self._range_owner.append(owner)
 
     def _stack_kernel_fits(self, nblocks, want_attn):
         heads_ok = self.H == 1 or (self.H == 2 and self.D == 64)
@@ -929,9 +964,10 @@
                     and L.lib.cr_stack_fwd_head_supported(last[2][0], C.byref(d), C.byref(n))):
                 self._keep += [d, n]
                 self.fwd[-1] = ("cr_stack_fwd_head", L.lib.cr_stack_fwd_head, (last[2][0], C.byref(d), C.byref(n)))
-                self._block_slab_range(pname + ".gamma", pname + ".beta", 2 * self.B)
+                self._block_slab_range(pname + ".gamma", pname + ".beta", 2 * self.B, owner="fwd")
                 return
             self._call(self.fwd, "cr_head_fwd_bwd_ln", C.byref(d), C.byref(n))
+            self._block_slab_range(pname + ".gamma", pname + ".beta", self.n_slabs, owner="fwd")
             return
         ds = self._grad_of(seq_emb)
         self._grad_written.add(id(ds))
@@ -1067,11 +1103,15 @@
                     per[a:b] = self.n_wslabs
             for a, b, c in self._block_bwd_ranges:
                 per[a:b] = c
-            if lay.n_dense and int(per.min()) < self.n_slabs:
-                nb = (lay.n_dense + 255) // 256
-                pad = np.zeros(nb * 256, np.int32)
-                pad[:lay.n_dense] = per
-                cnt = pad.reshape(nb, 256).max(1).astype(np.int32)
+            self.slab_fold_plan, cnt = self._plan_folds(per) if (self.slab_fold and lay.n_dense) else ({}, slab_block_counts(lay.n_dense, per))
+            if lay.n_dense and (int(per.min()) < self.n_slabs or self.slab_fold_plan):
+                for i, lst in self.slab_fold_plan.items():
+                    blocks = (C.c_int32 * len(lst))(*[k for k, _ in lst])
+                    cs = (C.c_int32 * len(lst))(*[c for _, c in lst])
+                    fd = L.SlabFoldDesc(self.Gs.data_ptr(), self.Gs.shape[1], blocks, cs, len(lst))
+                    self._keep += [blocks, cs, fd]
+                    name, _, args = self.bwd[i]
+                    self.bwd[i] = (name, L.lib.cr_stack_block_bwd_fold, args + (C.byref(fd),))
                 self.slab_counts = torch.from_numpy(cnt).to(self.dev)
                 counts = self.slab_counts.data_ptr()
             ad = L.AdamDesc(self.P.data_ptr(), self.Mom.data_ptr(), self.Vel.data_ptr(), self.Gt.data_ptr(), self.Gs.data_ptr(),
@@ -1097,6 +1137,17 @@
                              self.state.data_ptr(), self.Gflat.data_ptr() + 4 * lay.n_total, counts))
             self._l2 = ("cr_l2_penalty", L.lib.cr_l2_penalty, (self.P.data_ptr(), n_l2, 0.5 * l2, self.state.data_ptr())) if n_l2 else None
             self._keep += [ad, ad1]
+
+    def _plan_folds(self, per):
+        pos = {id(e): i for i, e in enumerate(self.bwd)}
+        known = []
+        for (a, b, _), owner in zip(self._block_bwd_ranges, self._range_owner):
+            if owner == "fwd":
+                known.append((a, b, -1))
+            elif owner and id(owner[0]) in pos:
+                known.append((a, b, pos[id(owner[0])]))
+        launches = [i for i, (name, _, _) in enumerate(self.bwd) if name == "cr_stack_block_bwd" and self.B <= self.n_slabs]
+        return plan_slab_folds(self.layout.n_dense, per, known, launches)
 
     def set_batch(self, seq, pos=None, neg=None, time=None, hours=None, days=None):
         limits = dict(seq=self.itemnum, pos=self.itemnum, neg=self.itemnum, time=self.hp.max_bins, hours=24, days=7)
@@ -1427,7 +1478,12 @@
             self.Gt.zero_()
             self._run([self._tgrad], torch.cuda.current_stream().cuda_stream)
             torch.cuda.synchronize()
-        flat = torch.cat([self.Gt, self.Gs.sum(0)[:self.layout.n_dense]]) / max(n, 1.0)
+        dense = torch.zeros(max(self.layout.n_dense, 1), dtype=torch.float32, device=self.dev)
+        if self.layout.n_dense:
+            L.check(L.lib.cr_reduce_slabs(self.Gs.data_ptr(), self.n_slabs, self.layout.n_dense, dense.data_ptr(), None, None,
+                                          self.slab_counts.data_ptr() if self.slab_counts is not None else None,
+                                          torch.cuda.current_stream().cuda_stream), "cr_reduce_slabs")
+        flat = torch.cat([self.Gt, dense[:self.layout.n_dense]]) / max(n, 1.0)
         return {k: self.layout.view(flat, k).clone() for k in self.layout.logical_names()}
 
     def n_launches(self):
diff --git a/context-aware-sequential-recommendation_amd/lib.py b/context-aware-sequential-recommendation_amd/lib.py
--- a/context-aware-sequential-recommendation_amd/lib.py
+++ b/context-aware-sequential-recommendation_amd/lib.py
@@ -97,6 +97,10 @@
 
 class BlockBwd1Ext(C.Structure):
     _fields_ = [("dy2", c_p), ("dx2", c_p), ("lnf_dy2", c_p), ("d_addend2", c_p)]
+
+
+class SlabFoldDesc(C.Structure):
+    _fields_ = [("slabs", c_p), ("slab_stride", c_i), ("blocks", C.POINTER(C.c_int32)), ("counts", C.POINTER(C.c_int32)), ("n_blocks", c_i)]
 
 
 class BlockTailDesc(C.Structure):
@@ -203,6 +207,8 @@
 _sig("cr_stack_block_bwd_deal", c_i, [c_i, c_i, C.POINTER(C.c_uint32)])
 _sig("cr_stack_block_bwd", c_i, [C.POINTER(BlockBwdDesc), C.POINTER(AttnDesc), C.POINTER(BlockBwd1Ext), C.POINTER(LnBwdDesc), C.POINTER(EmbedBwdDesc),
                                  c_i, c_i, c_i, c_p])
+_sig("cr_stack_block_bwd_fold", c_i, [C.POINTER(BlockBwdDesc), C.POINTER(AttnDesc), C.POINTER(BlockBwd1Ext), C.POINTER(LnBwdDesc), C.POINTER(EmbedBwdDesc),
+                                      c_i, c_i, c_i, C.POINTER(SlabFoldDesc), c_p])
 _sig("cr_block_ln_qkv_bwd_scatter", c_i, [C.POINTER(BlockBwdDesc), C.POINTER(EmbedBwdDesc), c_p])
 _sig("cr_wide_supported", c_i, [C.POINTER(BlockDesc), c_i])
 _sig("cr_wide_ln_qkv_fwd", c_i, [C.POINTER(BlockDesc), c_i, c_p])
@@ -246,7 +252,7 @@
 
 EXPORTS = ["cr_version", "cr_last_error", "cr_step_begin", "cr_ids_ring_next", "cr_embed_fwd", "cr_embed_bwd", "cr_layernorm_fwd",
            "cr_layernorm_bwd", "cr_gemm_rows", "cr_gemm_wgrad", "cr_eltwise", "cr_attn_fwd", "cr_attn_bwd",
-           "cr_block_ln_qkv_fwd", "cr_block_ln_qkv_fwd_gather", "cr_block_ln_ffn_fwd", "cr_block_ln_ffn_fwd_tail", "cr_stack_fwd_supported", "cr_stack_fwd", "cr_block_ln_ffn_bwd", "cr_block_ln_qkv_bwd", "cr_stack_bwd_supported", "cr_stack_ffn_bwd", "cr_stack_ffn_bwd_ln", "cr_stack_ffn_bwd_heads", "cr_stack_qkv_bwd", "cr_stack_qkv_bwd_scatter", "cr_stack_block_bwd_supported", "cr_stack_block_bwd", "cr_stack_block_bwd_deal", "cr_rows_pack", "cr_rows_add", "cr_block_ln_qkv_bwd_scatter",
+           "cr_block_ln_qkv_fwd", "cr_block_ln_qkv_fwd_gather", "cr_block_ln_ffn_fwd", "cr_block_ln_ffn_fwd_tail", "cr_stack_fwd_supported", "cr_stack_fwd", "cr_block_ln_ffn_bwd", "cr_block_ln_qkv_bwd", "cr_stack_bwd_supported", "cr_stack_ffn_bwd", "cr_stack_ffn_bwd_ln", "cr_stack_ffn_bwd_heads", "cr_stack_qkv_bwd", "cr_stack_qkv_bwd_scatter", "cr_stack_block_bwd_supported", "cr_stack_block_bwd", "cr_stack_block_bwd_fold", "cr_stack_block_bwd_deal", "cr_rows_pack", "cr_rows_add", "cr_block_ln_qkv_bwd_scatter",
            "cr_wide_supported", "cr_wide_ln_qkv_fwd", "cr_wide_ln_ffn_fwd", "cr_wide_ln_ffn_fwd_tail", "cr_wide_ln_ffn_bwd", "cr_wide_ln_qkv_bwd",
            "cr_head_fwd_bwd", "cr_head_fwd_bwd_ln", "cr_stack_fwd_head_supported", "cr_stack_fwd_head", "cr_test_logits", "cr_adam_step", "cr_reduce_slabs", "cr_l2_penalty", "cr_graph_begin", "cr_graph_end", "cr_graph_launch",
            "cr_graph_destroy", "cr_sampler_create", "cr_sampler_next", "cr_sampler_destroy",
diff --git a/include/castrec.h b/include/castrec.h
--- a/include/castrec.h
+++ b/include/castrec.h
@@ -224,6 +224,16 @@
 int cr_stack_block_bwd_supported(const cr_block_bwd_desc* d, const cr_attn_desc* ad, int B, int T, int precision);
 int cr_stack_block_bwd(const cr_block_bwd_desc* d, const cr_attn_desc* ad, const cr_block_bwd1_ext* x, const cr_ln_bwd_desc* lnf,
                        const cr_embed_bwd_desc* sc, int B, int T, int precision, void* stream);
+struct cr_slab_fold_desc {
+    float* slabs;
+    int slab_stride;
+    const int32_t* blocks;
+    const int32_t* counts;
+    int n_blocks;
+};
+typedef struct cr_slab_fold_desc cr_slab_fold_desc;
+int cr_stack_block_bwd_fold(const cr_block_bwd_desc* d, const cr_attn_desc* ad, const cr_block_bwd1_ext* x, const cr_ln_bwd_desc* lnf,
+                            const cr_embed_bwd_desc* sc, int B, int T, int precision, const cr_slab_fold_desc* fold, void* stream);
 int cr_stack_block_bwd_deal(int tiles, int query_pass, uint32_t* pk);
 
 int cr_wide_supported(const cr_block_desc* d, int precision);
```

After: 395,500 sequences/s. -4.3%, worse.
